# makezur/super_primitive

Hardware: AMD Instinct MI355X
Metric: GN iters/sec (640x480x64-seg frame pairs) (higher is better)
Workload: dtype f32; 1 GPU; Replica-shaped two-frame SfM, 640x480, 64 segments (grid, 4 px overlap), pyramid level 0 of a 3-level pyramid; BASELINE.json configs[1]; pairs_per_gpu=384, segment_pixels_per_pair=373056, optimiser=gn, tile_points=8192, span_points=4096, granule=64

## Files before the change

include/sp_hip.h:

```cpp
#ifndef SP_HIP_H
#define SP_HIP_H

#include <stdint.h>

#ifdef __cplusplus
extern "C" {
#endif

#define SP_ABI_VERSION 18

#define SP_EINVAL (-1)
#define SP_ELIMIT (-2)

#define SP_GRAD_PARTIAL_FLOATS 16
#define SP_GN_PARTIAL_FLOATS   32
#define SP_GNA_PARTIAL_FLOATS  48

int sp_abi_version(void);


int sp_mask_count(const uint8_t* masks, int N, int H, int W, int32_t* row_counts, int32_t* counts,
                  int32_t* seg_off, void* stream);

int sp_table_fill(const uint8_t* masks, const float* logdepth, const float* keypoints, int N, int H, int W,
                  const int32_t* seg_off, const int32_t* row_off, uint32_t* pix, float* baseL, float* kp_L,
                  void* stream);

int sp_table_sample_source(uint32_t* pix, const float* baseL, const int32_t* seg_off, const float* kp_L,
                           const float* kld, int N, int P, int H, int W, const float* img, int Hl, int Wl,
                           const float* K, float* src4, int set_validity, void* stream);

int sp_pack_rgb(const float* chw, int B, int H, int W, float* hwc3, void* stream);

int sp_blur_decimate(const float* in, int C, int H, int W, float* out, void* stream);

#define SP_PREP_MAX_STRIDES 4
#define SP_PREP_MAX_LEVELS 4
typedef struct SpPrepTable {
    const uint8_t* masks;
    const float* logdepth;
    const float* keypoints;
    float* kp_L;
    int32_t* row_counts[SP_PREP_MAX_STRIDES];
    int32_t* counts[SP_PREP_MAX_STRIDES];
    const int32_t* seg_off[SP_PREP_MAX_STRIDES];
    uint32_t* pix[SP_PREP_MAX_STRIDES];
    float* baseL[SP_PREP_MAX_STRIDES];
    int32_t stride[SP_PREP_MAX_STRIDES];
    int32_t N, H, W, n_strides;
    uint32_t* bits;
    const int32_t* boxes;
} SpPrepTable;
typedef struct SpPrepSample {
    uint32_t* pix;
    const float* baseL;
    const int32_t* seg_off;
    const int32_t* counts;
    const float* kp_L;
    const float* kld;
    const float* K;
    const float* image[SP_PREP_MAX_LEVELS];
    float* src4[SP_PREP_MAX_LEVELS];
    int32_t Hl[SP_PREP_MAX_LEVELS], Wl[SP_PREP_MAX_LEVELS];
    int32_t N, P, H, W, n_levels;
    int32_t granule;
} SpPrepSample;
#define SP_PREP_DEPTH_TABLE 0x10000
#define SP_PREP_DENSE_L 0x20000
typedef struct SpPrepImage {
    const float* in;
    float* out;
    int32_t H, W;
} SpPrepImage;
int sp_prepare_count(const SpPrepTable* tables, int n_tables, int max_rows, int max_N, void* stream);
int sp_prepare_count_boxed(const SpPrepTable* tables, int n_tables, int max_rows, int max_N, void* stream);
int sp_prepare_fill(const SpPrepTable* tables, int n_tables, int max_rows, int max_N, void* stream);
int sp_prepare_sample(const SpPrepSample* jobs, int n_jobs, int max_P, void* stream);
int sp_prepare_sample_pairs(const SpPrepSample* jobs_a, int max_P_a, const SpPrepSample* jobs_b, int max_P_b, int n_jobs, void* stream);
int sp_prepare_blur(const SpPrepImage* jobs, int n_jobs, int C, int max_out_pixels, void* stream);
int sp_prepare_pack(const SpPrepImage* jobs, int n_jobs, int max_pixels, void* stream);
typedef struct SpPrepImagePack {
    const float* in;
    float* out;
    float* packed_in;
    float* packed_out;
    int32_t H, W;
} SpPrepImagePack;
int sp_prepare_blur_pack(const SpPrepImagePack* jobs, int n_jobs, int max_out_pixels, void* stream);
int sp_prepare_gather(const float* const* src, const long long* off, int n, float* out, void* stream);

int sp_photo_cost_grad(const uint32_t* pix, const float* src4, const int32_t* seg_off, const float* kp_L,
                       const int32_t* tiles, const int32_t* seg_tile_off, int n_tiles, int N, int P, int H, int W,
                       const float* K_src, const float* kld, const float* trg3, int Hl, int Wl,
                       const float* K_trg, const float* pose, int B, const float* aff_src, const float* aff_trg,
                       float zmin, float* workspace, float* residual, float* g_kld, float* g_pose, float* g_aff,
                       void* stream);

int sp_points_workspace_floats(int n_points, int B);
int sp_points_cost_grad(const float* xyz, const float* rgb, int n_points, int P_total, int H, int W, const float* trg3,
                        int Hl, int Wl, const float* K_trg, const float* pose, int B, const float* aff_src,
                        const float* aff_trg, float zmin, float* workspace, float* residual, float* g_pose, float* g_aff,
                        void* stream);

int sp_photo_stats(const uint32_t* pix, const float* src4, const int32_t* seg_off, const float* kp_L, int N, int P,
                   int H, int W, const float* K_src, const float* kld, const float* trg3, int Hl, int Wl,
                   const float* K_trg, const float* pose, int B, const float* aff_src, const float* aff_trg,
                   float zmin, float* src_pts, float* trg_pts, float* src_rgb, float* trg_rgb, float* raw,
                   uint8_t* src_valid, uint8_t* trg_valid, int64_t* seg_ids, int stride, void* stream);

#define SP_GRAD_SEG_FLOATS 1
#define SP_GN_SEG_FLOATS 12
#define SP_GNA_SEG_FLOATS 12
typedef struct SpPair {
    const uint32_t* pix;
    const float*    src4;
    const float*    kp_L;
    const float*    trg3;
    float*          kld;
    float*          pose;
    float*          aff;
    const int32_t*  seg_tile_off;
    float K_src[4];
    float K_trg[4];
    int32_t N, P, H, W, Hl, Wl;
    int32_t tile0;
    int32_t n_tiles;
    float zmin;
    int32_t rec0;
} SpPair;

int sp_host_work_list_chunks(const long long* pc, int n_segs, int tile_points, int granule);
int sp_host_layout(const int32_t* counts, int n_lattices, int n_segs, const long long* n_off, int n_pairs, int granule,
                   long long* pc, long long* seg_pos, long long* p_off, int32_t* seg_off, long long* points);
int sp_host_work_list(const long long* pc, const long long* seg_pos, const long long* n_off, int n_pairs, int span_points,
                      int tile_points, int granule , int records_per_chunk ,
                      int32_t* chunks, int32_t* spans, int32_t* seg_tile_off, long long* sto_off, long long* c_off, long long* s_off);

#define SP_COST_WAVE_SPANS 0x100
#define SP_COST_DEPTH_TABLE 0x200

int sp_pairs_cost(const SpPair* pairs, const int32_t* chunks, const int32_t* spans, int n_spans, int mode, float irls_eps,
                  float* span_partials, float* seg_partials, void* stream);
struct SpRunDesc;
int sp_pairs_cost_opt(const SpPair* pairs, const int32_t* chunks, const int32_t* spans, int n_spans, int mode, float irls_eps,
                      float* span_partials, float* seg_partials, const int32_t* done, const uint32_t* pix_base,
                      const struct SpRunDesc* desc, void* stream);

int sp_pairs_adam_step(const SpPair* pairs, int n_pairs, int max_N, const float* span_partials, const float* seg_partials,
                       float lr_kld, float lr_pose, float lr_aff, float* state, float* losses, void* stream);

#define SP_LM_STATE_FLOATS 8
int sp_pairs_gn_step(const SpPair* pairs, int n_pairs, int max_N, const float* span_partials, const float* seg_partials,
                     float lm_up, float lm_down, float lm_min, float* lm_state, float* backup, float* costs, void* stream);

int sp_pairs_gn_step_conv(const SpPair* pairs, int n_pairs, int max_N, const float* span_partials, const float* seg_partials,
                          float lm_up, float lm_down, float lm_min, float* lm_state, float* backup, float* costs, float conv_tol,
                          int32_t* done, void* stream);

typedef struct SpRunDesc {
    uint32_t valid[2];
    float d[2];
    float base[2];
    float k;
    int32_t runs;
} SpRunDesc;

int sp_run_desc_build(const uint32_t* pix, int n_groups, SpRunDesc* desc, int32_t* n_general, void* stream);

#define SP_MAX_PHASES 12
#define SP_PHASE_POSE_ONLY 1
#define SP_PHASE_WAVE_SPANS 2
#define SP_PHASE_DEPTH_TABLE 4
#define SP_PHASE_DEPTH_DAMP_SHIFT 8
#define SP_PHASE_DEPTH_DAMP(k) (((k) & 0xff) << SP_PHASE_DEPTH_DAMP_SHIFT)
#define SP_PHASE_ADAM 8
#define SP_PHASE_PREDICTED_EXIT 16
typedef struct SpPhase {
    const SpPair* pairs;
    const int32_t* chunks;
    const int32_t* spans;
    float* span_partials;
    float* seg_partials;
    int32_t n_spans;
    int32_t max_iters;
    float irls_eps;
    float conv_tol;
    int32_t flags;
    int32_t next;
} SpPhase;
typedef struct SpSchedule {
    SpPhase phase[SP_MAX_PHASES];
    int32_t n_phases;
    int32_t entry;
    int32_t retry_entry;
    int32_t retry2_entry;
    float adam_lr_pose, adam_lr_kld;
    float* adam_state;
} SpSchedule;

#define SP_STATUS_NONFINITE   1
#define SP_STATUS_LAST_CAP    2
#define SP_STATUS_DEPTH_RANGE 4
#define SP_STATUS_COST        8
#define SP_STATUS_VALID       16
#define SP_STATUS_SEGMENTS    32
#define SP_STATUS_RETRIED     0x100
#define SP_STATUS_ADAM        0x400
#define SP_STATUS_UNFINISHED  0x200
#define SP_DIAG_FLOATS 8
typedef struct SpVerdict {
    int32_t* status;
    float* diag;
    int32_t* attempts;
    const float* pose0;
    const float* kld0;
    const float* pose_base;
    const float* kld_base;
    float kld_bound;
    float cost_bound;
    float cost_ratio;
    float valid_min;
    int32_t retry_mask;
    float lam0;
    float seg_max_ratio;
    float seg_mean_ratio;
    int32_t* evals;
    float seg_product;
    float pad_;
} SpVerdict;
#define SP_VERDICT_SEGMENTS 2048
#define SP_VERDICT_SEGMENT_POINTS 64
#define SP_VERDICT_MIN_SEGMENTS 8
int sp_pairs_schedule_cost(const SpSchedule* sched, const int32_t* phase, void* stream);
int sp_pairs_schedule_gn_step(const SpSchedule* sched, int n_pairs, int max_N, float lm_up, float lm_down, float lm_min,
                              float* lm_state, float* backup, float* costs, int32_t* phase, int32_t* iters, const SpVerdict* verdict ,
                              void* stream);

int sp_pairs_schedule_run(const SpSchedule* sched, int n_pairs, int max_N, float lm_up, float lm_down, float lm_min,
                          float* lm_state, float* backup, float* costs, int32_t* phase, int32_t* iters, int check_every,
                          int max_rounds, int32_t* flag_dev, int32_t* flag_host, const SpVerdict* verdict , void* stream);

typedef struct SpQueue {
    const SpPair* qpairs[SP_MAX_PHASES];
    SpPair* slot_pairs[SP_MAX_PHASES];
    int32_t max_spans[SP_MAX_PHASES];
    int32_t n_queue;
    int32_t pad_;
    int32_t* head;
    int32_t* slot_pair;
    float* q_costs;
    float* q_lm;
    float lam0;
    int32_t pad2_;
    int32_t* active;
} SpQueue;
int sp_pairs_schedule_run_queue(const SpSchedule* sched, const SpQueue* queue, int n_slots, int max_N, float lm_up, float lm_down,
                                float lm_min, float* lm_state, float* backup, float* costs, int32_t* phase, int32_t* iters,
                                int check_every, int max_rounds, int32_t* flag_dev, int32_t* flag_host, const SpVerdict* verdict ,
                                void* stream);

int sp_pairs_adam_iterate(const SpPair* pairs, const int32_t* chunks, const int32_t* spans, int n_spans, int n_pairs, int max_N,
                          float* span_partials, float* seg_partials, int32_t* arrivals, float lr_kld, float lr_pose, float lr_aff, float* state,
                          float* losses, void* stream);
int sp_pairs_gn_iterate(const SpPair* pairs, const int32_t* chunks, const int32_t* spans, int n_spans, int n_pairs, int max_N,
                        float irls_eps, float* span_partials, float* seg_partials, int32_t* arrivals, float lm_up, float lm_down,
                        float lm_min,
                        float* lm_state, float* backup, float* costs, void* stream);

typedef struct SpWindowNode {
    float T[16];
    float a[6];
    float m[6], v[6];
    float aff[2];
    float aff_m[2], aff_v[2];
    float lr_pose;
    float lr_aff;
    int32_t kind;
    int32_t flags;
} SpWindowNode;

typedef struct SpWindowEdge {
    int32_t src_node;
    int32_t trg_node;
    int32_t block;
    float weight;
} SpWindowEdge;

typedef struct SpWindowBlock {
    float* kld;
    float* m;
    float* v;
    int32_t N;
    float lr;
} SpWindowBlock;

int sp_window_scratch_doubles(int n_edges, int max_N);

int sp_window_compose(const SpPair* pairs, const SpWindowEdge* edges, int n_edges, SpWindowNode* nodes, int n_nodes, void* stream);

int sp_window_step(const SpPair* pairs, const SpWindowEdge* edges, int n_edges, SpWindowNode* nodes, int n_nodes,
                   const SpWindowBlock* blocks, int n_blocks, int max_N, const float* span_partials, const float* seg_partials,
                   double* scratch, int abs_loss, int skip_first, float rel_tol, float* state, float* losses, int max_losses,
                   void* stream);

int sp_window_gn_scratch_doubles(int n_edges, int n_blocks, int sum_N, int max_N, int n_unknowns);
int sp_window_gn_profile_offset(int n_edges, int n_blocks, int sum_N, int max_N, int n_unknowns);
int sp_window_gn_step(const SpPair* pairs, const SpWindowEdge* edges, int n_edges, SpWindowNode* nodes, int n_nodes,
                      const SpWindowBlock* blocks, int n_blocks, int sum_N, int max_N, int n_unknowns, const float* span_partials,
                      const float* seg_partials, double* scratch, SpWindowNode* nodes_backup, float* kld_backup, int flags,
                      float lm_up, float lm_down, float lm_min, float conv_tol, float* state, float* losses, int max_losses,
                      void* stream);

typedef struct SpWindowGn {
    const SpPair* pairs;
    const int32_t* chunks;
    const int32_t* spans;
    const SpWindowEdge* edges;
    SpWindowNode* nodes;
    const SpWindowBlock* blocks;
    float* span_partials;
    float* seg_partials;
    double* scratch;
    SpWindowNode* nodes_backup;
    float* kld_backup;
    float* state;
    float* losses;
    int32_t n_spans, n_edges, n_nodes, n_blocks, sum_N, max_N, n_unknowns, max_losses;
} SpWindowGn;
int sp_window_gn_multi_bytes(void);
int sp_window_gn_run_multi(const SpWindowGn* windows, int n_windows, float irls_eps, int flags, float lm_up, float lm_down, float lm_min,
                           float conv_tol, int max_iters, int check_every, void* args_dev, float* states_dev, float* states_host, void* stream);

int sp_window_gn_run(const SpPair* pairs, const int32_t* chunks, const int32_t* spans, int n_spans, float irls_eps,
                     const SpWindowEdge* edges, int n_edges, SpWindowNode* nodes, int n_nodes, const SpWindowBlock* blocks, int n_blocks,
                     int sum_N, int max_N, int n_unknowns, float* span_partials, float* seg_partials, double* scratch,
                     SpWindowNode* nodes_backup, float* kld_backup, int flags, float lm_up, float lm_down, float lm_min, float conv_tol,
                     float* state, float* losses, int max_losses, int max_iters, int check_every, float* state_host, void* stream);


int sp_depth_expand(const uint8_t* masks, const float* logdepth, const float* keypoints, const float* kld, int N,
                    int H, int W, int log_space, float* out, void* stream);

int sp_depth_splat(const uint32_t* pix, const float* baseL, const int32_t* seg_off, const float* kp_L,
                   const float* kld, int N, int P, int H, int W, const float* K, const float* pose,
                   unsigned long long* keys, float* out, void* stream);

int sp_depth_splat_mean(const uint32_t* pix, const float* baseL, const int32_t* seg_off, const float* kp_L, const float* kld, int N,
                        int P, int H, int W, const float* K, const float* pose, void* acc, float* out, void* stream);

int sp_segment_reinit(const uint32_t* pix, const float* baseL, const int32_t* seg_off, const float* kp_L, int N,
                      int P, int H, int W, const float* est_depth, int mode, float* scratch, float* out_kld,
                      uint8_t* out_visible, void* stream);

int sp_depth_average(const uint32_t* pix, const float* baseL, const int32_t* seg_off, const float* kp_L,
                     const float* kld, const uint8_t* visible, int N, int P, int H, int W, void* acc,
                     float* out_depth, uint8_t* out_invalid, void* stream);

int sp_depth_accumulate(const uint32_t* pix, const float* baseL, const int32_t* seg_off, const float* kp_L,
                        const float* kld, const uint8_t* visible, int N, int P, int H, int W, void* acc, void* stream);
int sp_depth_average_finish(const void* acc, int H, int W, float* out_depth, uint8_t* out_invalid, void* stream);

int sp_se3_retract(const float* a, const float* X, int n, float* T, const float* grad_T, float* grad_a, void* stream);

int sp_renormalise_se3(float* T, int n, void* stream);


int sp_depth_discontinuity(const float* logdepth, const uint8_t* valid, int N, int H, int W, int filter_size,
                           float threshold, float* scratch, uint8_t* split, uint8_t* disc, void* stream);

int sp_label_components(const uint8_t* fg, int N, int H, int W, int32_t* parent, int32_t* labels, int32_t* sizes,
                        void* stream);

int sp_collect_parts(const int32_t* labels, const int32_t* sizes, const uint8_t* masks, const uint8_t* split, int N, int H,
                     int W, int cap, int32_t* parts, int32_t* n_parts, int32_t* bg_sizes, void* stream);

int sp_build_part_masks(const uint8_t* masks, const uint8_t* split, const int32_t* labels, int H, int W,
                        const int32_t* parts, int K, uint8_t* out, void* stream);

int sp_kth_mask_pixel(const uint8_t* masks, const int32_t* row_off, int K, int H, int W, const int32_t* kth,
                      int32_t* out_rc, void* stream);

int sp_normal_integration_plan_words(int N);
int sp_normal_integration_segment_floats(int H, int W);
int sp_normal_integration_plan(const uint8_t* masks, const int32_t* boxes_or_null, int N, int H, int W, int32_t* plan, void* stream);
int sp_normal_integration(const float* normals, const float* K, const uint8_t* masks, const int32_t* boxes_or_null, int N, int H,
                          int W, int cg_max_iter, float cg_tol, int flags, float* scratch, long long scratch_floats, float* depth,
                          float* info, void* stream);

int sp_depth_fill_workspace_bytes(int B, int H, int W);
int sp_depth_fill_nearest(const float* depth, const uint8_t* invalid, int B, int H, int W, void* workspace, float* filled,
                          int32_t* index_or_null, int32_t* counts, void* stream);
int sp_depth_metrics_workspace_doubles(int B, int H, int W);
int sp_depth_metrics(const float* estimate, const float* target, const uint8_t* valid, int B, int H, int W, double* workspace,
                     double* out, void* stream);

int sp_kf_criterion(const float* depth, int n, float thresh, const float* pose_src, const float* pose_trg, float* out,
                    void* stream);
int sp_kf_criterion_ws_words(void);
int sp_kf_criterion_ws(const float* depth, int n, float thresh, const float* pose_src, const float* pose_trg, uint32_t* ws, float* out,
                       void* stream);

#define SP_CHAIN_LEVELS 4
#define SP_CHAIN_PHASES 6
#define SP_CHAIN_TRACK 1
#define SP_CHAIN_SUPP 2
#define SP_CHAIN_CRITERION 4
typedef struct SpChainPhase {
    int32_t level;
    int32_t max_iters;
    float irls_eps, conv_tol;
} SpChainPhase;
typedef struct SpChainWindow {
    SpWindowGn gn[SP_CHAIN_LEVELS];
    SpChainPhase phase[SP_CHAIN_PHASES];
    int32_t n_phases;
    int32_t check_every;
    int32_t flags;
    float lam0;
    float lm_up, lm_down, lm_min;
    int32_t check_first;
    float* state_host;
} SpChainWindow;
typedef struct SpChainTarget {
    float* packed[SP_CHAIN_LEVELS];
    const float* pose;
    const float* aff;
    int32_t node;
    int32_t pad_;
} SpChainTarget;
typedef struct SpChainStep {
    int32_t stages;
    int32_t H, W, n_levels;
    const float* image;
    float* level[SP_CHAIN_LEVELS];
    SpChainWindow track;
    SpChainTarget track_target;
    float* out_pose;
    float* out_aff;
    SpChainWindow supp;
    SpChainTarget supp_target[2];
    int32_t supp_images;
    int32_t kld_n;
    const float* kld_src;
    float* kld_dst;
    const uint32_t* pix; const float* baseL; const int32_t* seg_off; const float* kp_L; const float* kld;
    const float* K; const float* kf_pose;
    int32_t N, P;
    unsigned long long* keys; float* depth_out;
    float* rel_pose;
    float* crit;
    uint32_t* crit_ws;
    float* crit_host;
    float valid_thresh;
    int32_t track_iters, supp_iters;
    int32_t pad_;
} SpChainStep;

int sp_chain_multi_bytes(void);
int sp_chain_step_multi(SpChainStep* steps, int n_steps, void* args_dev, float* states_dev, float* states_host, void* stream);

#ifdef __cplusplus
}
#endif
#endif
```

super_primitive_amd/_lib.py:

```python
from __future__ import annotations

import ctypes
import os
from ctypes import c_float, c_int, c_void_p

_HERE = os.path.dirname(os.path.abspath(__file__))
LIB_PATH = os.environ.get("SP_HIP_LIB") or os.path.join(_HERE, "csrc", "libsp_hip.so")

P = c_void_p
I = c_int
F = c_float

SIGNATURES = {
    "sp_abi_version": [],
    "sp_mask_count": [P, I, I, I, P, P, P, P],
    "sp_table_fill": [P, P, P, I, I, I, P, P, P, P, P, P],
    "sp_table_sample_source": [P, P, P, P, P, I, I, I, I, P, I, I, P, P, I, P],
    "sp_pack_rgb": [P, I, I, I, P, P],
    "sp_blur_decimate": [P, I, I, I, P, P],
    "sp_photo_cost_grad": [P, P, P, P, P, P, I, I, I, I, I, P, P, P, I, I, P, P, I, P, P, F, P, P, P, P, P, P],
    "sp_points_workspace_floats": [I, I],
    "sp_points_cost_grad": [P, P, I, I, I, I, P, I, I, P, P, I, P, P, F, P, P, P, P, P],
    "sp_photo_stats": [P, P, P, P, I, I, I, I, P, P, P, I, I, P, P, I, P, P, F, P, P, P, P, P, P, P, P, I, P],
    "sp_pairs_cost": [P, P, P, I, I, F, P, P, P],
    "sp_pairs_adam_step": [P, I, I, P, P, F, F, F, P, P, P],
    "sp_pairs_gn_step": [P, I, I, P, P, F, F, F, P, P, P, P],
    "sp_pairs_cost_opt": [P, P, P, I, I, F, P, P, P, P, P, P],
    "sp_run_desc_build": [P, I, P, P, P],
    "sp_pairs_gn_step_conv": [P, I, I, P, P, F, F, F, P, P, P, F, P, P],
    "sp_prepare_count": [P, I, I, I, P],
    "sp_prepare_count_boxed": [P, I, I, I, P],
    "sp_prepare_fill": [P, I, I, I, P],
    "sp_prepare_sample": [P, I, I, P],
    "sp_prepare_sample_pairs": [P, I, P, I, I, P],
    "sp_prepare_blur": [P, I, I, I, P],
    "sp_prepare_pack": [P, I, I, P],
    "sp_prepare_blur_pack": [P, I, I, P],
    "sp_prepare_gather": [P, P, I, P, P],
    "sp_host_work_list_chunks": [P, I, I, I],
    "sp_host_layout": [P, I, I, P, I, I, P, P, P, P, P],
    "sp_host_work_list": [P, P, P, I, I, I, I, I, P, P, P, P, P, P],
    "sp_pairs_schedule_cost": [P, P, P],
    "sp_pairs_schedule_gn_step": [P, I, I, F, F, F, P, P, P, P, P, P, P],
    "sp_pairs_schedule_run": [P, I, I, F, F, F, P, P, P, P, P, I, I, P, P, P, P],
    "sp_pairs_schedule_run_queue": [P, P, I, I, F, F, F, P, P, P, P, P, I, I, P, P, P, P],
    "sp_pairs_adam_iterate": [P, P, P, I, I, I, P, P, P, F, F, F, P, P, P],
    "sp_pairs_gn_iterate": [P, P, P, I, I, I, F, P, P, P, F, F, F, P, P, P, P],
    "sp_window_scratch_doubles": [I, I],
    "sp_window_compose": [P, P, I, P, I, P],
    "sp_window_step": [P, P, I, P, I, P, I, I, P, P, P, I, I, F, P, P, I, P],
    "sp_window_gn_scratch_doubles": [I, I, I, I, I],
    "sp_window_gn_profile_offset": [I, I, I, I, I],
    "sp_window_gn_run": [P, P, P, I, F, P, I, P, I, P, I, I, I, I, P, P, P, P, P, I, F, F, F, F, P, P, I, I, I, P, P],
    "sp_window_gn_multi_bytes": [],
    "sp_window_gn_run_multi": [P, I, F, I, F, F, F, F, I, I, P, P, P, P],
    "sp_window_gn_step": [P, P, I, P, I, P, I, I, I, I, P, P, P, P, P, I, F, F, F, F, P, P, I, P],
    "sp_depth_expand": [P, P, P, P, I, I, I, I, P, P],
    "sp_depth_splat_mean": [P, P, P, P, P, I, I, I, I, P, P, P, P, P],
    "sp_depth_splat": [P, P, P, P, P, I, I, I, I, P, P, P, P, P],
    "sp_segment_reinit": [P, P, P, P, I, I, I, I, P, I, P, P, P, P],
    "sp_depth_average": [P, P, P, P, P, P, I, I, I, I, P, P, P, P],
    "sp_depth_accumulate": [P, P, P, P, P, P, I, I, I, I, P, P],
    "sp_depth_average_finish": [P, I, I, P, P, P],
    "sp_kf_criterion": [P, I, F, P, P, P, P],
    "sp_chain_multi_bytes": [],
    "sp_chain_step_multi": [P, I, P, P, P, P],
    "sp_kf_criterion_ws_words": [],
    "sp_kf_criterion_ws": [P, I, F, P, P, P, P, P],
    "sp_se3_retract": [P, P, I, P, P, P, P],
    "sp_renormalise_se3": [P, I, P],
    "sp_depth_discontinuity": [P, P, I, I, I, I, F, P, P, P, P],
    "sp_label_components": [P, I, I, I, P, P, P, P],
    "sp_collect_parts": [P, P, P, P, I, I, I, I, P, P, P, P],
    "sp_build_part_masks": [P, P, P, I, I, P, I, P, P],
    "sp_kth_mask_pixel": [P, P, I, I, I, P, P, P],
    "sp_normal_integration_plan_words": [I],
    "sp_normal_integration_segment_floats": [I, I],
    "sp_normal_integration_plan": [P, P, I, I, I, P, P],
    "sp_normal_integration": [P, P, P, P, I, I, I, I, F, I, P, ctypes.c_longlong, P, P, P],
    "sp_depth_fill_workspace_bytes": [I, I, I],
    "sp_depth_fill_nearest": [P, P, I, I, I, P, P, P, P, P],
    "sp_depth_metrics_workspace_doubles": [I, I, I],
    "sp_depth_metrics": [P, P, P, I, I, I, P, P, P],
}

SP_ABI_VERSION = 18
SP_GRAD_PARTIAL_FLOATS = 16
SP_GN_PARTIAL_FLOATS = 32
SP_GNA_PARTIAL_FLOATS = 48
SP_GNA_SEG_FLOATS = 12
SP_GRAD_SEG_FLOATS = 1
SP_GN_SEG_FLOATS = 12
SP_LM_STATE_FLOATS = 8


class SpPair(ctypes.Structure):
    _fields_ = [
        ("pix", c_void_p), ("src4", c_void_p), ("kp_L", c_void_p), ("trg3", c_void_p),
        ("kld", c_void_p), ("pose", c_void_p), ("aff", c_void_p), ("seg_tile_off", c_void_p),
        ("K_src", c_float * 4), ("K_trg", c_float * 4),
        ("N", c_int), ("P", c_int), ("H", c_int), ("W", c_int), ("Hl", c_int), ("Wl", c_int),
        ("tile0", c_int), ("n_tiles", c_int), ("zmin", c_float), ("rec0", c_int),
    ]


SP_MAX_PHASES = 12
SP_PHASE_POSE_ONLY = 1
SP_PHASE_WAVE_SPANS = 2
SP_COST_WAVE_SPANS = 0x100
SP_COST_DEPTH_TABLE = 0x200
SP_PHASE_DEPTH_TABLE = 4
SP_PHASE_ADAM = 8
SP_PHASE_PREDICTED_EXIT = 16
SP_PHASE_DEPTH_DAMP_SHIFT = 8
SP_PREP_DEPTH_TABLE = 0x10000
SP_PREP_DENSE_L = 0x20000


SP_PREP_MAX_STRIDES = 4
SP_PREP_MAX_LEVELS = 4


class SpPrepTable(ctypes.Structure):
    _fields_ = [("masks", c_void_p), ("logdepth", c_void_p), ("keypoints", c_void_p), ("kp_L", c_void_p),
                ("row_counts", c_void_p * SP_PREP_MAX_STRIDES), ("counts", c_void_p * SP_PREP_MAX_STRIDES),
                ("seg_off", c_void_p * SP_PREP_MAX_STRIDES), ("pix", c_void_p * SP_PREP_MAX_STRIDES),
                ("baseL", c_void_p * SP_PREP_MAX_STRIDES), ("stride", c_int * SP_PREP_MAX_STRIDES),
                ("N", c_int), ("H", c_int), ("W", c_int), ("n_strides", c_int), ("bits", c_void_p), ("boxes", c_void_p)]


class SpPrepSample(ctypes.Structure):
    _fields_ = [("pix", c_void_p), ("baseL", c_void_p), ("seg_off", c_void_p), ("counts", c_void_p), ("kp_L", c_void_p), ("kld", c_void_p),
                ("K", c_void_p), ("image", c_void_p * SP_PREP_MAX_LEVELS), ("src4", c_void_p * SP_PREP_MAX_LEVELS),
                ("Hl", c_int * SP_PREP_MAX_LEVELS), ("Wl", c_int * SP_PREP_MAX_LEVELS),
                ("N", c_int), ("P", c_int), ("H", c_int), ("W", c_int), ("n_levels", c_int), ("granule", c_int)]


class SpPrepImage(ctypes.Structure):
    _fields_ = [("inp", c_void_p), ("out", c_void_p), ("H", c_int), ("W", c_int)]


class SpPrepImagePack(ctypes.Structure):
    _fields_ = [("inp", c_void_p), ("out", c_void_p), ("packed_in", c_void_p), ("packed_out", c_void_p), ("H", c_int), ("W", c_int)]


class SpPhase(ctypes.Structure):
    _fields_ = [("pairs", c_void_p), ("chunks", c_void_p), ("spans", c_void_p), ("span_partials", c_void_p), ("seg_partials", c_void_p),
                ("n_spans", c_int), ("max_iters", c_int), ("irls_eps", c_float), ("conv_tol", c_float), ("flags", c_int), ("next", c_int)]


class SpSchedule(ctypes.Structure):
    _fields_ = [("phase", SpPhase * SP_MAX_PHASES), ("n_phases", c_int), ("entry", c_int), ("retry_entry", c_int), ("retry2_entry", c_int),
                ("adam_lr_pose", c_float), ("adam_lr_kld", c_float), ("adam_state", c_void_p)]


SP_STATUS_NONFINITE = 1
SP_STATUS_LAST_CAP = 2
SP_STATUS_DEPTH_RANGE = 4
SP_STATUS_COST = 8
SP_STATUS_VALID = 16
SP_STATUS_SEGMENTS = 32
SP_STATUS_RETRIED = 0x100
SP_STATUS_UNFINISHED = 0x200
SP_STATUS_ADAM = 0x400
SP_STATUS_FAILED = SP_STATUS_NONFINITE | SP_STATUS_LAST_CAP | SP_STATUS_DEPTH_RANGE | SP_STATUS_COST | SP_STATUS_VALID | SP_STATUS_SEGMENTS | SP_STATUS_UNFINISHED
SP_VERDICT_SEGMENTS = 2048
SP_VERDICT_SEGMENT_POINTS = 64
SP_VERDICT_MIN_SEGMENTS = 8
SP_DIAG_FLOATS = 8


class SpVerdict(ctypes.Structure):
    _fields_ = [("status", c_void_p), ("diag", c_void_p), ("attempts", c_void_p), ("pose0", c_void_p), ("kld0", c_void_p),
                ("pose_base", c_void_p), ("kld_base", c_void_p), ("kld_bound", c_float), ("cost_bound", c_float), ("cost_ratio", c_float),
                ("valid_min", c_float), ("retry_mask", c_int), ("lam0", c_float), ("seg_max_ratio", c_float), ("seg_mean_ratio", c_float), ("evals", c_void_p),
                ("seg_product", c_float), ("pad_", c_float)]


class SpQueue(ctypes.Structure):
    _fields_ = [("qpairs", c_void_p * SP_MAX_PHASES), ("slot_pairs", c_void_p * SP_MAX_PHASES), ("max_spans", c_int * SP_MAX_PHASES),
                ("n_queue", c_int), ("pad_", c_int),
                ("head", c_void_p), ("slot_pair", c_void_p), ("q_costs", c_void_p), ("q_lm", c_void_p), ("lam0", c_float), ("pad2_", c_int),
                ("active", c_void_p)]


class SpWindowGn(ctypes.Structure):
    _fields_ = [("pairs", c_void_p), ("chunks", c_void_p), ("spans", c_void_p), ("edges", c_void_p), ("nodes", c_void_p), ("blocks", c_void_p),
                ("span_partials", c_void_p), ("seg_partials", c_void_p), ("scratch", c_void_p), ("nodes_backup", c_void_p), ("kld_backup", c_void_p),
                ("state", c_void_p), ("losses", c_void_p), ("n_spans", c_int), ("n_edges", c_int), ("n_nodes", c_int), ("n_blocks", c_int),
                ("sum_N", c_int), ("max_N", c_int), ("n_unknowns", c_int), ("max_losses", c_int)]


SP_CHAIN_LEVELS, SP_CHAIN_PHASES = 4, 6
SP_CHAIN_TRACK, SP_CHAIN_SUPP, SP_CHAIN_CRITERION = 1, 2, 4


class SpChainPhase(ctypes.Structure):
    _fields_ = [("level", c_int), ("max_iters", c_int), ("irls_eps", c_float), ("conv_tol", c_float)]


class SpChainWindow(ctypes.Structure):
    _fields_ = [("gn", SpWindowGn * SP_CHAIN_LEVELS), ("phase", SpChainPhase * SP_CHAIN_PHASES), ("n_phases", c_int), ("check_every", c_int),
                ("flags", c_int), ("lam0", c_float), ("lm_up", c_float), ("lm_down", c_float), ("lm_min", c_float), ("check_first", c_int),
                ("state_host", c_void_p)]


class SpChainTarget(ctypes.Structure):
    _fields_ = [("packed", c_void_p * SP_CHAIN_LEVELS), ("pose", c_void_p), ("aff", c_void_p), ("node", c_int), ("pad_", c_int)]


class SpChainStep(ctypes.Structure):
    _fields_ = [("stages", c_int), ("H", c_int), ("W", c_int), ("n_levels", c_int), ("image", c_void_p), ("level", c_void_p * SP_CHAIN_LEVELS),
                ("track", SpChainWindow), ("track_target", SpChainTarget), ("out_pose", c_void_p), ("out_aff", c_void_p),
                ("supp", SpChainWindow), ("supp_target", SpChainTarget * 2), ("supp_images", c_int), ("kld_n", c_int), ("kld_src", c_void_p),
                ("kld_dst", c_void_p),
                ("pix", c_void_p), ("baseL", c_void_p), ("seg_off", c_void_p), ("kp_L", c_void_p), ("kld", c_void_p), ("K", c_void_p),
                ("kf_pose", c_void_p), ("N", c_int), ("P", c_int), ("keys", c_void_p), ("depth_out", c_void_p), ("rel_pose", c_void_p),
                ("crit", c_void_p), ("crit_ws", c_void_p), ("crit_host", c_void_p), ("valid_thresh", c_float), ("track_iters", c_int), ("supp_iters", c_int),
                ("pad_", c_int)]


class SpWindowNode(ctypes.Structure):
    _fields_ = [("T", c_float * 16), ("a", c_float * 6), ("m", c_float * 6), ("v", c_float * 6), ("aff", c_float * 2),
                ("aff_m", c_float * 2), ("aff_v", c_float * 2), ("lr_pose", c_float), ("lr_aff", c_float),
                ("kind", c_int), ("flags", c_int)]


class SpWindowEdge(ctypes.Structure):
    _fields_ = [("src_node", c_int), ("trg_node", c_int), ("block", c_int), ("weight", c_float)]


class SpWindowBlock(ctypes.Structure):
    _fields_ = [("kld", c_void_p), ("m", c_void_p), ("v", c_void_p), ("N", c_int), ("lr", c_float)]


_lib = None


def load():
    global _lib
    if _lib is not None:
        return _lib
    if not os.path.exists(LIB_PATH):
        raise RuntimeError(
            f"{LIB_PATH} not found: build it with `python -c 'import __graft_entry__ as g; g.build()'` "
            "(hipcc --offload-arch=gfx950).  There is no CPU / PyTorch fallback for the hot path.")
    try:
        import torch
    except Exception:
        pass
    lib = ctypes.CDLL(LIB_PATH)
    for name, args in SIGNATURES.items():
        fn = getattr(lib, name)
        fn.argtypes = args
        fn.restype = c_int
    if lib.sp_abi_version() != SP_ABI_VERSION:
        raise RuntimeError("libsp_hip.so ABI version mismatch; rebuild")
    _lib = lib
    return lib


def check(rc, what):
    if rc != 0:
        kind = {-1: "SP_EINVAL (bad argument)", -2: "SP_ELIMIT (size not supported)"}.get(rc, f"hipError_t {rc}")
        raise RuntimeError(f"{what} failed: {kind}")


def ptr(t):
    return None if t is None else ctypes.c_void_p(t.data_ptr())


_raw_stream = None


def stream_ptr():
    global _raw_stream
    if _raw_stream is None:
        import torch
        raw, cur = getattr(torch._C, "_cuda_getCurrentRawStream", None), getattr(torch._C, "_cuda_getDevice", None)
        if raw is not None and cur is not None:
            _raw_stream = lambda: raw(cur())
        else:
            _raw_stream = lambda: torch.cuda.current_stream().cuda_stream
    return ctypes.c_void_p(_raw_stream())


def require_device(*tensors):
    import torch
    dev = None
    for t in tensors:
        if t is None:
            continue
        if not t.is_cuda:
            raise RuntimeError("super_primitive_amd: the photometric hot path is HIP-only; got a CPU tensor. "
                               "Move the keyframe to a cuda device (no CPU fallback exists).")
        if dev is None:
            dev = t.device
        elif t.device != dev:
            raise RuntimeError(f"super_primitive_amd: operands on different devices ({dev} and {t.device})")
    if dev is not None and dev.index is not None and dev.index != torch.cuda.current_device():
        raise RuntimeError(f"super_primitive_amd: operands live on {dev} but the current device is "
                           f"cuda:{torch.cuda.current_device()}; wrap the call in `with torch.cuda.device({dev.index}):` "
                           "(one process per GPU is the supported layout)")
```

super_primitive_amd/csrc/sp_solve_device.h:

```cpp
#pragma once
#include "sp_device.h"

#define SP_LM_STRIDE SP_LM_STATE_FLOATS

template <int NV>
__device__ __forceinline__ void reduce_columns(const float* __restrict__ p, int n_tiles, double* out, double* scratch) {
    constexpr int G = SP_BLOCK / NV;
    const int g = threadIdx.x / NV, c = threadIdx.x - g * NV;
    if (g < G) {
        double s = 0.0;
        for (int t = g; t < n_tiles; t += 8 * G) {
            float v[8];
#pragma unroll
            for (int u = 0; u < 8; ++u) {
                const int tt = t + u * G;
                const float x = p[(size_t)min(tt, n_tiles - 1) * NV + c];
                v[u] = tt < n_tiles ? x : 0.f;
            }
#pragma unroll
            for (int u = 0; u < 8; ++u) s += (double)v[u];
        }
        scratch[g * NV + c] = s;
    }
    __syncthreads();
    if (threadIdx.x < NV) {
        double s = 0.0;
#pragma unroll
        for (int k = 0; k < G; ++k) s += scratch[k * NV + threadIdx.x];
        out[threadIdx.x] = s;
    }
    __syncthreads();
}

__device__ void se3_retract_left(const double xi[6], float* T16) {
    const double wx = xi[3], wy = xi[4], wz = xi[5];
    const double th2 = wx * wx + wy * wy + wz * wz;
    double A, B, C;
    if (th2 < 1e-12) {
        A = 1.0 - th2 / 6.0; B = 0.5 - th2 / 24.0; C = 1.0 / 6.0 - th2 / 120.0;
    } else if (th2 < 1e-4) {
        A = 1.0 - th2 / 6.0 * (1.0 - th2 / 20.0);
        B = 0.5 - th2 / 24.0 * (1.0 - th2 / 30.0);
        C = 1.0 / 6.0 - th2 / 120.0 * (1.0 - th2 / 42.0);
    } else {
        const double th = sqrt(th2);
        const double sn = sin(th), cs = cos(th);
        A = sn / th; B = (1.0 - cs) / th2; C = (th - sn) / (th2 * th);
    }
    const double W[9] = {0, -wz, wy, wz, 0, -wx, -wy, wx, 0};
    double W2[9];
    for (int i = 0; i < 3; ++i)
        for (int j = 0; j < 3; ++j) W2[3 * i + j] = W[3 * i] * W[j] + W[3 * i + 1] * W[3 + j] + W[3 * i + 2] * W[6 + j];
    double E[9], V[9];
    for (int i = 0; i < 9; ++i) {
        const double I = (i % 4 == 0) ? 1.0 : 0.0;
        E[i] = I + A * W[i] + B * W2[i];
        V[i] = I + B * W[i] + C * W2[i];
    }
    double dt[3];
    for (int i = 0; i < 3; ++i) dt[i] = V[3 * i] * xi[0] + V[3 * i + 1] * xi[1] + V[3 * i + 2] * xi[2];
    double R[9], t[3];
    for (int i = 0; i < 3; ++i) {
        for (int j = 0; j < 3; ++j) R[3 * i + j] = T16[4 * i + j];
        t[i] = T16[4 * i + 3];
    }
    for (int i = 0; i < 3; ++i) {
        for (int j = 0; j < 3; ++j)
            T16[4 * i + j] = (float)(E[3 * i] * R[j] + E[3 * i + 1] * R[3 + j] + E[3 * i + 2] * R[6 + j]);
        T16[4 * i + 3] = (float)(E[3 * i] * t[0] + E[3 * i + 1] * t[1] + E[3 * i + 2] * t[2] + dt[i]);
    }
    T16[12] = 0.f; T16[13] = 0.f; T16[14] = 0.f; T16[15] = 1.f;
}

__device__ __forceinline__ float adam_torch(float g, float& m, float& v, float neg_step, float bc2s) {
    m = m + 0.1f * (g - m);
    v = v * 0.999f;
    v = v + 0.001f * g * g;
    const float denom = sqrtf(v) / bc2s + 1e-8f;
    return neg_step * (m / denom);
}

struct AdamArgs {
    int max_N;
    float lr_kld, lr_pose, lr_aff;
    float* state;
    float* losses;
};

__device__ __forceinline__ void solve_adam(const SpPair* __restrict__ pairs, int pi, const float* __restrict__ partials,
                                           const float* __restrict__ seg_partials, const AdamArgs& h) {
    const int max_N = h.max_N;
    const float lr_kld = h.lr_kld, lr_pose = h.lr_pose, lr_aff = h.lr_aff;
    float* __restrict__ state = h.state;
    float* __restrict__ losses = h.losses;
    constexpr int NV = SP_GRAD_PARTIAL_FLOATS;
    __shared__ double sums[NV];
    __shared__ double scratch[(SP_BLOCK / NV) * NV];
    const SpPair& pr = pairs[pi];
    const float* p = partials + (size_t)pr.tile0 * NV;
    reduce_columns<NV>(p, pr.n_tiles, sums, scratch);
    const double scale = 1.0 / (3.0 * (double)pr.P);
    const float residual = (float)(sums[0] * scale);
    const double up = residual > 0.f ? scale : (residual < 0.f ? -scale : 0.0);
    float* st = state + (size_t)pi * (2 + 2 * (max_N + 8));
    float* m_kld = st + 2; float* v_kld = m_kld + max_N;
    float* m_xi = v_kld + max_N; float* v_xi = m_xi + 6;
    float* m_af = v_xi + 6; float* v_af = m_af + 2;
    const float step = st[0] + 1.f;
    const double bc1 = 1.0 - pow(0.9, (double)step);
    const float bc2s = (float)sqrt(1.0 - pow(0.999, (double)step));
    const float ns_kld = (float)(-(double)lr_kld / bc1), ns_pose = (float)(-(double)lr_pose / bc1), ns_aff = (float)(-(double)lr_aff / bc1);
    __syncthreads();
    for (int n = threadIdx.x; n < pr.N; n += SP_BLOCK) {
        double s = 0.0;
        const float* sp = seg_partials + (size_t)pr.rec0 * SP_GRAD_SEG_FLOATS;
        const int t0 = pr.seg_tile_off[n], t1 = pr.seg_tile_off[n + 1];
        for (int t = t0; t < t1; t += 8) {
            float v[8];
#pragma unroll
            for (int u = 0; u < 8; ++u) v[u] = sp[(size_t)min(t + u, t1 - 1) * SP_GRAD_SEG_FLOATS];
#pragma unroll
            for (int u = 0; u < 8; ++u) s += (t + u < t1) ? (double)v[u] : 0.0;
        }
        const float g = (float)(s * up);
        pr.kld[n] += adam_torch(g, m_kld[n], v_kld[n], ns_kld, bc2s);
    }
    if (threadIdx.x == 0) {
        double gR[9], gt[3], R[9], t[3];
        for (int i = 0; i < 3; ++i) {
            gt[i] = sums[1 + i] * up;
            for (int j = 0; j < 3; ++j) { gR[3 * i + j] = sums[4 + 3 * i + j] * up; R[3 * i + j] = pr.pose[4 * i + j]; }
            t[i] = pr.pose[4 * i + 3];
        }
        double A[9];
        for (int i = 0; i < 3; ++i)
            for (int j = 0; j < 3; ++j)
                A[3 * i + j] = R[3 * i] * gR[3 * j] + R[3 * i + 1] * gR[3 * j + 1] + R[3 * i + 2] * gR[3 * j + 2] + t[i] * gt[j];
        const float g6[6] = {(float)gt[0], (float)gt[1], (float)gt[2],
                             (float)(A[5] - A[7]), (float)(A[6] - A[2]), (float)(A[1] - A[3])};
        double xi[6];
        for (int i = 0; i < 6; ++i) xi[i] = adam_torch(g6[i], m_xi[i], v_xi[i], ns_pose, bc2s);
        se3_retract_left(xi, pr.pose);
        if (pr.aff) {
            const float ga = (float)(sums[14] * up), gb = (float)(sums[15] * up);
            pr.aff[2] += adam_torch(ga, m_af[0], v_af[0], ns_aff, bc2s);
            pr.aff[3] += adam_torch(gb, m_af[1], v_af[1], ns_aff, bc2s);
        }
        st[0] = step;
        losses[pi] = fabsf(residual);
    }
}


__device__ bool ldlt6_solve(double S[36], double rhs[6]) {
    double dinv[6];
    for (int j = 0; j < 6; ++j) {
        double d = S[7 * j];
        for (int k = 0; k < j; ++k) d -= S[6 * j + k] * S[6 * j + k] * S[7 * k];
        if (!(d > 0.0)) return false;
        S[7 * j] = d;
        dinv[j] = 1.0 / d;
        for (int i = j + 1; i < 6; ++i) {
            double v = S[6 * i + j];
            for (int k = 0; k < j; ++k) v -= S[6 * i + k] * S[6 * j + k] * S[7 * k];
            S[6 * i + j] = v * dinv[j];
        }
    }
    for (int i = 0; i < 6; ++i) {
        double v = rhs[i];
        for (int k = 0; k < i; ++k) v -= S[6 * i + k] * rhs[k];
        rhs[i] = v;
    }
    for (int i = 0; i < 6; ++i) rhs[i] *= dinv[i];
    for (int i = 5; i >= 0; --i) {
        double v = rhs[i];
        for (int k = i + 1; k < 6; ++k) v -= S[6 * k + i] * rhs[k];
        rhs[i] = v;
    }
    return true;
}

#define SP_SEG_CACHE 256

__device__ __forceinline__ void segment_system(const float* __restrict__ p, const int32_t* __restrict__ seg_tile_off, int n,
                                               double lam, double (&o)[8], bool pose_only = false) {
    constexpr int NV = SP_GN_SEG_FLOATS;
    if (pose_only) {
#pragma unroll
        for (int i = 0; i < 8; ++i) o[i] = 0.0;
        return;
    }
    double h[6] = {0, 0, 0, 0, 0, 0}, D = 0.0, bd = 0.0;
    const int t0 = seg_tile_off[n], t1 = seg_tile_off[n + 1];
    for (int t = t0; t < t1; t += 8) {
        float v[8][8];
#pragma unroll
        for (int u = 0; u < 8; ++u) {
            const float4* q = reinterpret_cast<const float4*>(p + (size_t)min(t + u, t1 - 1) * NV);
            const float4 a = q[0], b = q[1];
            v[u][0] = a.x; v[u][1] = a.y; v[u][2] = a.z; v[u][3] = a.w;
            v[u][4] = b.x; v[u][5] = b.y; v[u][6] = b.z; v[u][7] = b.w;
        }
#pragma unroll
        for (int u = 0; u < 8; ++u) {
            if (t + u < t1) {
#pragma unroll
                for (int i = 0; i < 6; ++i) h[i] += (double)v[u][i];
                D += (double)v[u][6];
                bd += (double)v[u][7];
            }
        }
    }
    const double Dd = D * (1.0 + lam);
#pragma unroll
    for (int i = 0; i < 6; ++i) o[i] = h[i];
    o[6] = Dd > 1e-12 ? 1.0 / Dd : 0.0;
    o[7] = bd;
}

struct GnArgs {
    int max_N;
    float lm_up, lm_down, lm_min;
    float* lm_state;
    float* backup;
    float* costs;
    float conv_tol;
    int32_t* done;
    int32_t* phase;
    int32_t* iters;
    int max_iters;
    int pose_only;
    int next_phase;
    float depth_damp;
    float adam_lr_pose, adam_lr_kld;
    float* adam_state;
    int predicted_exit;
    uint32_t idle_mask;
};

__device__ __forceinline__ void leave_phase(const GnArgs& h, int pi, float* __restrict__ ls, int spent, bool on_cap) {
    h.phase[pi] = h.next_phase;
    h.iters[pi] = 0;
    ls[1] = -1.f;
    ls[7] = on_cap ? (float)spent : -(float)spent;
}

__device__ __forceinline__ void solve_gn(const SpPair* __restrict__ pairs, int pi, const float* __restrict__ partials,
                                         const float* __restrict__ seg_partials, const GnArgs& h) {
    const int max_N = h.max_N;
    const float lm_up = h.lm_up, lm_down = h.lm_down, lm_min = h.lm_min;
    float* __restrict__ lm_state = h.lm_state;
    float* __restrict__ backup = h.backup;
    float* __restrict__ costs = h.costs;
    constexpr int NV = SP_GN_PARTIAL_FLOATS;
    __shared__ double sums[NV];
    __shared__ double scratch[(SP_BLOCK / NV) * NV];
    __shared__ double seg[SP_SEG_CACHE][8];
    __shared__ double schur_part[8][27];
    __shared__ double schur[27];
    __shared__ double dxi[6];
    __shared__ double gain_part[SP_WAVES];
    __shared__ int decision;
    const SpPair& pr = pairs[pi];
    if (h.done && h.done[pi]) return;
    const float* p = partials + (size_t)pr.tile0 * NV;
    const float* sp = seg_partials + (size_t)pr.rec0 * SP_GN_SEG_FLOATS;
    float* ls = lm_state + (size_t)pi * SP_LM_STRIDE;
    float* bk = backup + (size_t)pi * (16 + max_N);
    reduce_columns<NV>(p, pr.n_tiles, sums, scratch);
    const double cost = sums[0] / (3.0 * (double)pr.P);
    if (threadIdx.x == 0) {
        const float last = ls[1];
        int rej = 0;
        if (last >= 0.f && (float)cost > last * (1.f + 1e-6f) && ls[4] == 0.f) rej = 1;
        if (!rej && (h.done || h.phase) && h.conv_tol > 0.f && last >= 0.f && ls[4] == 0.f && (last - (float)cost) <= h.conv_tol * last) {
            rej = 2;
            if (h.done) h.done[pi] = 1;
            if (h.phase) { leave_phase(h, pi, ls, h.iters[pi], false); ls[4] = 0.f; }
        }
        decision = rej;
        ls[5] = (float)cost;
        ls[6] = (float)(sums[28] / (double)pr.P);
        costs[pi] = (float)cost;
    }
    __syncthreads();
    if (decision == 2) return;
    if (decision == 1) {
        for (int i = threadIdx.x; i < 16; i += SP_BLOCK) pr.pose[i] = bk[i];
        for (int n = threadIdx.x; n < pr.N; n += SP_BLOCK) pr.kld[n] = bk[16 + n];
        if (threadIdx.x == 0) {
            ls[0] *= lm_up; ls[3] += 1.f; ls[4] = 1.f;
            if (h.phase) {
                const int n = h.iters[pi] + 1;
                if (n >= h.max_iters) { leave_phase(h, pi, ls, n, true); ls[4] = 0.f; }
                else h.iters[pi] = n;
            }
        }
        return;
    }
    float lambda = ls[0];
    if (ls[4] == 0.f) lambda = fmaxf(lambda * lm_down, lm_min);
    const double lam = (double)lambda;
    for (int i = threadIdx.x; i < 16; i += SP_BLOCK) bk[i] = pr.pose[i];
    for (int n = threadIdx.x; n < pr.N; n += SP_BLOCK) bk[16 + n] = pr.kld[n];
    const int n_cached = min(pr.N, SP_SEG_CACHE);
    for (int n = threadIdx.x; n < n_cached; n += SP_BLOCK) {
        double o[8];
        segment_system(sp, pr.seg_tile_off, n, lam + (double)h.depth_damp, o, h.pose_only != 0);
#pragma unroll
        for (int i = 0; i < 8; ++i) seg[n][i] = o[i];
    }
    __syncthreads();
    {
        const int k = threadIdx.x >> 3, j = threadIdx.x & 7;
        if (k < 27) {
            int a = 0, b = 0;
            if (k < 21) { int rem = k, row = 0; while (rem >= 6 - row) { rem -= 6 - row; ++row; } a = row; b = row + rem; }
            else a = k - 21;
            double acc = 0.0;
            for (int n = j; n < pr.N; n += 8) {
                double o[8];
                if (n < SP_SEG_CACHE) {
#pragma unroll
                    for (int i = 0; i < 8; ++i) o[i] = seg[n][i];
                } else segment_system(sp, pr.seg_tile_off, n, lam + (double)h.depth_damp, o, h.pose_only != 0);
                acc += o[a] * (k < 21 ? o[b] : o[7]) * o[6];
            }
            schur_part[j][k] = acc;
        }
    }
    __syncthreads();
    if (threadIdx.x < 27) {
        double v = 0.0;
#pragma unroll
        for (int j = 0; j < 8; ++j) v += schur_part[j][threadIdx.x];
        schur[threadIdx.x] = v;
    }
    __syncthreads();
    if (threadIdx.x == 0) {
        double S[36], rhs[6];
        int k = 0;
        for (int i = 0; i < 6; ++i)
            for (int j = i; j < 6; ++j) {
                double v = sums[1 + k] - schur[k];
                if (i == j) v += lam * sums[1 + k] + 1e-12;
                S[6 * i + j] = v; S[6 * j + i] = v;
                ++k;
            }
        for (int i = 0; i < 6; ++i) rhs[i] = -(sums[22 + i] - schur[21 + i]);
        const bool ok = ldlt6_solve(S, rhs);
        for (int i = 0; i < 6; ++i) dxi[i] = ok ? rhs[i] : 0.0;
        ls[0] = lambda; ls[1] = (float)cost; ls[2] += 1.f; ls[4] = 0.f;
    }
    __syncthreads();
    double gain = 0.0;
    for (int n = threadIdx.x; n < pr.N; n += SP_BLOCK) {
        double o[8];
        if (n < SP_SEG_CACHE) {
#pragma unroll
            for (int i = 0; i < 8; ++i) o[i] = seg[n][i];
        } else segment_system(sp, pr.seg_tile_off, n, lam + (double)h.depth_damp, o, h.pose_only != 0);
        if (o[6] > 0.0) {
            double r = -o[7];
#pragma unroll
            for (int i = 0; i < 6; ++i) r -= o[i] * dxi[i];
            double dd = r * o[6];
            dd = fmin(fmax(dd, -0.5), 0.5);
            pr.kld[n] += (float)dd;
            gain -= o[7] * dd;
        }
    }
    if (threadIdx.x == 64) {
        double xi[6];
        for (int i = 0; i < 6; ++i) xi[i] = dxi[i];
        se3_retract_left(xi, pr.pose);
    }
    if (h.phase) {
#pragma unroll
        for (int o = 32; o > 0; o >>= 1) gain += __shfl_xor(gain, o, 64);
        if ((threadIdx.x & 63) == 0) gain_part[threadIdx.x >> 6] = gain;
        __syncthreads();
        if (threadIdx.x == 0) {
            const int n = h.iters[pi] + 1;
            bool done = false;
            if (h.predicted_exit && h.conv_tol > 0.f && h.depth_damp == 0.f && lambda <= 1e-2f) {
                double g = gain_part[0] + gain_part[1] + gain_part[2] + gain_part[3];
                for (int i = 0; i < 6; ++i) g -= sums[22 + i] * dxi[i];
                done = g / (3.0 * (double)pr.P) <= (double)h.conv_tol * cost;
            }
            if (done) leave_phase(h, pi, ls, n, false);
            else if (n >= h.max_iters) leave_phase(h, pi, ls, n, true);
            else h.iters[pi] = n;
        }
    }
}

__device__ __forceinline__ void solve_adam_sched(const SpPair* __restrict__ pairs, int pi, const float* __restrict__ partials,
                                                 const float* __restrict__ seg_partials, const GnArgs& h) {
    constexpr int NV = SP_GN_PARTIAL_FLOATS;
    __shared__ double sums[NV];
    __shared__ double scratch[(SP_BLOCK / NV) * NV];
    const SpPair& pr = pairs[pi];
    const int max_N = h.max_N;
    const float* p = partials + (size_t)pr.tile0 * NV;
    const float* sp = seg_partials + (size_t)pr.rec0 * SP_GN_SEG_FLOATS;
    float* ls = h.lm_state + (size_t)pi * SP_LM_STRIDE;
    reduce_columns<NV>(p, pr.n_tiles, sums, scratch);
    const double scale = 1.0 / (3.0 * (double)pr.P);
    float* st = h.adam_state + (size_t)pi * (2 + 2 * (max_N + 8));
    float* m_kld = st + 2; float* v_kld = m_kld + max_N;
    float* m_xi = v_kld + max_N; float* v_xi = m_xi + 6;
    const float step = st[0] + 1.f;
    const double bc1 = 1.0 - pow(0.9, (double)step);
    const float bc2s = (float)sqrt(1.0 - pow(0.999, (double)step));
    const float ns_kld = (float)(-(double)h.adam_lr_kld / bc1), ns_pose = (float)(-(double)h.adam_lr_pose / bc1);
    __syncthreads();
    for (int n = threadIdx.x; n < pr.N; n += SP_BLOCK) {
        double o[8];
        segment_system(sp, pr.seg_tile_off, n, 0.0, o);
        const float g = (float)(o[7] * scale);
        pr.kld[n] += adam_torch(g, m_kld[n], v_kld[n], ns_kld, bc2s);
    }
    if (threadIdx.x == 0) {
        double xi[6];
        for (int i = 0; i < 6; ++i) xi[i] = adam_torch((float)(sums[22 + i] * scale), m_xi[i], v_xi[i], ns_pose, bc2s);
        se3_retract_left(xi, pr.pose);
        st[0] = step;
        const float cost = (float)(sums[0] * scale);
        ls[1] = cost; ls[2] += 1.f; ls[4] = 0.f; ls[5] = cost;
        ls[6] = (float)(sums[28] / (double)pr.P);
        h.costs[pi] = cost;
        const int n = h.iters[pi] + 1;
        if (n >= h.max_iters) leave_phase(h, pi, ls, n, true);
        else h.iters[pi] = n;
    }
}

__device__ __forceinline__ void renormalise_rotation(float* __restrict__ M) {
    const float m00 = M[0], m01 = M[1], m02 = M[2], m10 = M[4], m11 = M[5], m12 = M[6], m20 = M[8], m21 = M[9], m22 = M[10];
    float q0 = 1.f + m00 + m11 + m22, q1 = 1.f + m00 - m11 - m22, q2 = 1.f - m00 + m11 - m22, q3 = 1.f - m00 - m11 + m22;
    q0 = q0 > 0.f ? sqrtf(q0) : 0.f; q1 = q1 > 0.f ? sqrtf(q1) : 0.f;
    q2 = q2 > 0.f ? sqrtf(q2) : 0.f; q3 = q3 > 0.f ? sqrtf(q3) : 0.f;
    int best = 0; float qb = q0;
    if (q1 > qb) { best = 1; qb = q1; }
    if (q2 > qb) { best = 2; qb = q2; }
    if (q3 > qb) { best = 3; qb = q3; }
    const float a = m21 - m12, b = m02 - m20, c = m10 - m01, d = m10 + m01, e = m02 + m20, f = m12 + m21;
    const float c0 = best == 0 ? q0 * q0 : (best == 1 ? a : (best == 2 ? b : c));
    const float c1 = best == 0 ? a : (best == 1 ? q1 * q1 : (best == 2 ? d : e));
    const float c2 = best == 0 ? b : (best == 1 ? d : (best == 2 ? q2 * q2 : f));
    const float c3 = best == 0 ? c : (best == 1 ? e : (best == 2 ? f : q3 * q3));
    const float den = 2.f * fmaxf(qb, 0.1f);
    const float r = c0 / den, x = c1 / den, y = c2 / den, z = c3 / den;
    const float s = 2.f / (r * r + x * x + y * y + z * z);
    M[0] = 1.f - s * (y * y + z * z); M[1] = s * (x * y - z * r);       M[2] = s * (x * z + y * r);
    M[4] = s * (x * y + z * r);       M[5] = 1.f - s * (x * x + z * z); M[6] = s * (y * z - x * r);
    M[8] = s * (x * z - y * r);       M[9] = s * (y * z + x * r);       M[10] = 1.f - s * (x * x + y * y);
}

template <int ND>
struct Dual {
    float v;
    float d[ND];
};
template <int ND> __device__ __forceinline__ Dual<ND> dconst(float c) { Dual<ND> r; r.v = c; for (int i = 0; i < ND; ++i) r.d[i] = 0.f; return r; }
template <int ND> __device__ __forceinline__ Dual<ND> operator+(const Dual<ND>& a, const Dual<ND>& b) { Dual<ND> r; r.v = a.v + b.v; for (int i = 0; i < ND; ++i) r.d[i] = a.d[i] + b.d[i]; return r; }
template <int ND> __device__ __forceinline__ Dual<ND> operator-(const Dual<ND>& a, const Dual<ND>& b) { Dual<ND> r; r.v = a.v - b.v; for (int i = 0; i < ND; ++i) r.d[i] = a.d[i] - b.d[i]; return r; }
template <int ND> __device__ __forceinline__ Dual<ND> operator-(const Dual<ND>& a) { Dual<ND> r; r.v = -a.v; for (int i = 0; i < ND; ++i) r.d[i] = -a.d[i]; return r; }
template <int ND> __device__ __forceinline__ Dual<ND> operator*(const Dual<ND>& a, const Dual<ND>& b) { Dual<ND> r; r.v = a.v * b.v; for (int i = 0; i < ND; ++i) r.d[i] = a.d[i] * b.v + a.v * b.d[i]; return r; }
template <int ND> __device__ __forceinline__ Dual<ND> operator*(float a, const Dual<ND>& b) { Dual<ND> r; r.v = a * b.v; for (int i = 0; i < ND; ++i) r.d[i] = a * b.d[i]; return r; }
template <int ND> __device__ __forceinline__ Dual<ND> chain(const Dual<ND>& a, float f, float df) { Dual<ND> r; r.v = f; for (int i = 0; i < ND; ++i) r.d[i] = df * a.d[i]; return r; }

template <int ND>
__device__ void se3_exp_times(const Dual<ND> (&a)[6], const float* __restrict__ X16, Dual<ND> (&T)[12]) {
    const Dual<ND> th2 = a[3] * a[3] + a[4] * a[4] + a[5] * a[5];
    const float t2 = th2.v;
    float A, B, C, dA, dB, dC;
    {
        const double t = (double)t2;
        double a_, b_, c_, da_, db_, dc_;
        if (t < 0.5) {
            double ia[10], ib[10], ic[10];
            {
                double f = 1.0;
                for (int k = 0; k < 10; ++k) {
                    const double n1 = 2.0 * k + 1.0;
                    if (k > 0) f *= (2.0 * k) * n1;
                    ia[k] = 1.0 / f; ib[k] = ia[k] / (n1 + 1.0); ic[k] = ib[k] / (n1 + 2.0);
                }
            }
            double va = 0.0, vb = 0.0, vc = 0.0, wa = 0.0, wb = 0.0, wc = 0.0;
            for (int k = 9; k >= 0; --k) {
                const double sg = (k & 1) ? -1.0 : 1.0;
                wa = wa * t + va; va = va * t + sg * ia[k];
                wb = wb * t + vb; vb = vb * t + sg * ib[k];
                wc = wc * t + vc; vc = vc * t + sg * ic[k];
            }
            a_ = va; b_ = vb; c_ = vc; da_ = wa; db_ = wb; dc_ = wc;
        } else {
            const double th = sqrt(t), sn = sin(th), cs = cos(th);
            a_ = sn / th; b_ = (1.0 - cs) / t; c_ = (th - sn) / (t * th);
            da_ = (cs * th - sn) / (2.0 * t * th);
            db_ = (sn * th - 2.0 * (1.0 - cs)) / (2.0 * t * t);
            dc_ = ((1.0 - cs) * th - 3.0 * (th - sn)) / (2.0 * t * t * th);
        }
        A = (float)a_; B = (float)b_; C = (float)c_; dA = (float)da_; dB = (float)db_; dC = (float)dc_;
    }
    const Dual<ND> dA_ = chain(th2, A, dA), dB_ = chain(th2, B, dB), dC_ = chain(th2, C, dC);
    const Dual<ND> z = dconst<ND>(0.f), one = dconst<ND>(1.f);
    const Dual<ND> W[9] = {z, -a[5], a[4], a[5], z, -a[3], -a[4], a[3], z};
    Dual<ND> W2[9];
    for (int i = 0; i < 3; ++i)
        for (int j = 0; j < 3; ++j) W2[3 * i + j] = W[3 * i] * W[j] + W[3 * i + 1] * W[3 + j] + W[3 * i + 2] * W[6 + j];
    Dual<ND> E[9], V[9];
    for (int i = 0; i < 9; ++i) {
        const Dual<ND> I = (i % 4 == 0) ? one : z;
        E[i] = I + dA_ * W[i] + dB_ * W2[i];
        V[i] = I + dB_ * W[i] + dC_ * W2[i];
    }
    for (int i = 0; i < 3; ++i) {
        const Dual<ND> dt = V[3 * i] * a[0] + V[3 * i + 1] * a[1] + V[3 * i + 2] * a[2];
        for (int j = 0; j < 3; ++j)
            T[4 * i + j] = X16[j] * E[3 * i] + X16[4 + j] * E[3 * i + 1] + X16[8 + j] * E[3 * i + 2];
        T[4 * i + 3] = X16[3] * E[3 * i] + X16[7] * E[3 * i + 1] + X16[11] * E[3 * i + 2] + dt;
    }
}
```

super_primitive_amd/csrc/sp_solver.hip:

```cpp
#include "sp_solve_device.h"

namespace {

__global__ __launch_bounds__(SP_BLOCK) void k_pairs_adam(const SpPair* __restrict__ pairs, const float* __restrict__ partials,
                                                         const float* __restrict__ seg_partials, AdamArgs h) {
    solve_adam(pairs, blockIdx.x, partials, seg_partials, h);
}

__global__ __launch_bounds__(SP_BLOCK) void k_pairs_gn(const SpPair* __restrict__ pairs, const float* __restrict__ partials,
                                                       const float* __restrict__ seg_partials, GnArgs h) {
    solve_gn(pairs, blockIdx.x, partials, seg_partials, h);
}

static_assert(sizeof(SpPhase) == 64 && sizeof(SpSchedule) == 800 && sizeof(SpVerdict) == 104 && sizeof(SpQueue) == 296 && sizeof(SpPair) == 136,
              "SpSchedule / SpVerdict / SpQueue / SpPair are part of the ABI");

__global__ __launch_bounds__(SP_BLOCK) void k_pairs_gn_sched(SpSchedule sched, GnArgs h, SpQueue q, SpVerdict v, const int32_t* __restrict__ active) {
    const int slot = active ? active[blockIdx.x] : blockIdx.x;
    const int ph = h.phase[slot];
    if (ph >= sched.n_phases || ph < 0) return;
    if ((h.idle_mask >> ph) & 1u) return;
    if (v.evals && threadIdx.x == 0) v.evals[(size_t)(q.n_queue > 0 ? q.slot_pair[slot] : slot) * SP_MAX_PHASES + ph] += 1;
    {
        const SpPhase& s = sched.phase[ph];
        h.conv_tol = s.conv_tol;
        h.max_iters = s.max_iters;
        h.pose_only = s.flags & SP_PHASE_POSE_ONLY;
        h.next_phase = s.next > 0 ? s.next : ph + 1;
        h.depth_damp = 0.125f * (float)((s.flags >> SP_PHASE_DEPTH_DAMP_SHIFT) & 0xff);
        h.adam_lr_pose = sched.adam_lr_pose; h.adam_lr_kld = sched.adam_lr_kld; h.adam_state = sched.adam_state;
        h.predicted_exit = s.flags & SP_PHASE_PREDICTED_EXIT;
        if ((s.flags & SP_PHASE_ADAM) && sched.adam_state) solve_adam_sched(s.pairs, slot, s.span_partials, s.seg_partials, h);
        else solve_gn(s.pairs, slot, s.span_partials, s.seg_partials, h);
    }
    if (q.n_queue <= 0 && !v.status) return;
    __shared__ int next_s, retry_s;
    __shared__ float dmax_s[SP_WAVES];
    __shared__ int bad_s[SP_WAVES];
    __shared__ float segc_s[SP_VERDICT_SEGMENTS];
    __shared__ float seg_med_s, seg_max_s[SP_WAVES];
    __shared__ int seg_n_s[SP_WAVES];
    __syncthreads();
    const int pid = q.n_queue > 0 ? q.slot_pair[slot] : slot;
    float* ls = h.lm_state + (size_t)slot * SP_LM_STRIDE;
    if (v.diag && threadIdx.x == 0) {
        float* first = v.diag + (size_t)pid * SP_DIAG_FLOATS + 5;
        if (*first == 0.f) *first = h.costs[slot];
    }
    if (h.phase[slot] < sched.n_phases) return;
    if (v.status) {
        const SpPair& pr = sched.phase[ph].pairs[slot];
        const float* kld0 = v.kld0 + (pr.kld - v.kld_base);
        const float* pose0 = v.pose0 + (pr.pose - v.pose_base);
        float dmax = 0.f;
        int bad = 0;
        for (int n = threadIdx.x; n < pr.N; n += SP_BLOCK) {
            const float d = fabsf(pr.kld[n] - kld0[n]);
            if (!(d <= 3.0e38f)) bad = 1;
            else dmax = fmaxf(dmax, d);
        }
        if (threadIdx.x < 12 && !(fabsf(pr.pose[threadIdx.x]) <= 3.0e38f)) bad = 1;
        const int n_seg = min(pr.N, SP_VERDICT_SEGMENTS);
        float smax = 0.f;
        int sn = 0;
        {
            const float* sp = sched.phase[ph].seg_partials + (size_t)pr.rec0 * SP_GN_SEG_FLOATS;
            for (int n = threadIdx.x; n < n_seg; n += SP_BLOCK) {
                double a = 0.0, c = 0.0;
                for (int t = pr.seg_tile_off[n]; t < pr.seg_tile_off[n + 1]; ++t) {
                    a += (double)sp[(size_t)t * SP_GN_SEG_FLOATS + 8];
                    c += (double)sp[(size_t)t * SP_GN_SEG_FLOATS + 9];
                }
                const float sc = c >= (double)SP_VERDICT_SEGMENT_POINTS ? (float)(a / (3.0 * c)) : -1.f;
                segc_s[n] = sc;
                if (sc >= 0.f) { smax = fmaxf(smax, sc); ++sn; }
            }
        }
#pragma unroll
        for (int o = 32; o > 0; o >>= 1) {
            dmax = fmaxf(dmax, __shfl_xor(dmax, o, 64)); bad |= __shfl_xor(bad, o, 64);
            smax = fmaxf(smax, __shfl_xor(smax, o, 64)); sn += __shfl_xor(sn, o, 64);
        }
        if ((threadIdx.x & 63) == 0) { dmax_s[threadIdx.x >> 6] = dmax; bad_s[threadIdx.x >> 6] = bad; seg_max_s[threadIdx.x >> 6] = smax; seg_n_s[threadIdx.x >> 6] = sn; }
        if (threadIdx.x == 0) seg_med_s = 0.f;
        __syncthreads();
        {
            const int n_judged = seg_n_s[0] + seg_n_s[1] + seg_n_s[2] + seg_n_s[3];
            const int want = (n_judged - 1) >> 1;
            for (int n = threadIdx.x; n < n_seg && n_judged >= SP_VERDICT_MIN_SEGMENTS; n += SP_BLOCK) {
                const float x = segc_s[n];
                if (x < 0.f) continue;
                int rank = 0;
                for (int j = 0; j < n_seg; ++j) {
                    const float y = segc_s[j];
                    rank += (y >= 0.f && (y < x || (y == x && j < n))) ? 1 : 0;
                }
                if (rank == want) seg_med_s = x;
            }
        }
        __syncthreads();
        if (threadIdx.x == 0) {
            dmax = fmaxf(fmaxf(dmax_s[0], dmax_s[1]), fmaxf(dmax_s[2], dmax_s[3]));
            bad = bad_s[0] | bad_s[1] | bad_s[2] | bad_s[3];
            const float cost = ls[5], first = v.diag ? v.diag[(size_t)pid * SP_DIAG_FLOATS + 5] : 0.f;
            int st = 0;
            if (bad || !(fabsf(cost) <= 3.0e38f)) st |= SP_STATUS_NONFINITE;
            if (ls[7] > 0.f) st |= SP_STATUS_LAST_CAP;
            if (v.kld_bound > 0.f && dmax > v.kld_bound) st |= SP_STATUS_DEPTH_RANGE;
            if ((v.cost_bound > 0.f && cost > v.cost_bound) || (v.cost_ratio > 0.f && first > 0.f && cost > v.cost_ratio * first)) st |= SP_STATUS_COST;
            if (v.valid_min > 0.f && ls[6] < v.valid_min) st |= SP_STATUS_VALID;
            const float seg_med = seg_med_s, seg_max = fmaxf(fmaxf(seg_max_s[0], seg_max_s[1]), fmaxf(seg_max_s[2], seg_max_s[3]));
            if (seg_med > 0.f && ((v.seg_max_ratio > 0.f && seg_max > v.seg_max_ratio * seg_med) || (v.seg_mean_ratio > 0.f && cost > v.seg_mean_ratio * seg_med) ||
                                  (v.seg_product > 0.f && (cost / seg_med - 1.f) * (seg_max / seg_med) > v.seg_product)))
                st |= SP_STATUS_SEGMENTS;
            const int attempt = v.attempts ? v.attempts[pid] : 2;
            const bool failed = (st & v.retry_mask) != 0;
            const bool has1 = sched.retry_entry >= 0 && sched.retry_entry < sched.n_phases, has2 = sched.retry2_entry >= 0 && sched.retry2_entry < sched.n_phases;
            int again = 0;
            if (failed && attempt == 0 && has1) again = 1;
            else if (failed && attempt <= 1 && has2) again = 2;
            retry_s = again;
            if (again) {
                v.attempts[pid] = again;
                h.phase[slot] = again == 1 ? sched.retry_entry : sched.retry2_entry; h.iters[slot] = 0;
                ls[0] = v.lam0; ls[1] = -1.f; ls[4] = 0.f; ls[7] = 0.f;
                if (v.diag) v.diag[(size_t)pid * SP_DIAG_FLOATS + 5] = 0.f;
            } else {
                v.status[pid] = st | (attempt > 0 && v.attempts ? SP_STATUS_RETRIED : 0) | (attempt > 1 && v.attempts ? SP_STATUS_ADAM : 0);
                if (v.diag) {
                    float* d = v.diag + (size_t)pid * SP_DIAG_FLOATS;
                    d[0] = cost; d[1] = dmax; d[2] = ls[6]; d[3] = fabsf(ls[7]); d[4] = (float)(v.attempts ? attempt + 1 : 1); d[6] = seg_med; d[7] = seg_max;
                }
            }
        }
        __syncthreads();
        if (retry_s) {
            for (int n = threadIdx.x; n < pr.N; n += SP_BLOCK) pr.kld[n] = kld0[n];
            if (threadIdx.x < 16) pr.pose[threadIdx.x] = pose0[threadIdx.x];
            if (sched.adam_state) {
                float* st = sched.adam_state + (size_t)slot * (2 + 2 * (h.max_N + 8));
                for (int i = threadIdx.x; i < 2 + 2 * (h.max_N + 8); i += SP_BLOCK) st[i] = 0.f;
            }
            return;
        }
    }
    if (q.n_queue <= 0) return;
    if (threadIdx.x < SP_LM_STRIDE) q.q_lm[(size_t)pid * SP_LM_STRIDE + threadIdx.x] = ls[threadIdx.x];
    if (threadIdx.x == 0) {
        q.q_costs[pid] = h.costs[slot];
        next_s = atomicAdd(q.head, 1);
    }
    __syncthreads();
    const int next = next_s;
    if (next >= q.n_queue) return;
    {
        constexpr int WORDS = (int)(sizeof(SpPair) / sizeof(uint32_t));
        for (int i = threadIdx.x; i < sched.n_phases * WORDS; i += SP_BLOCK) {
            const int p = i / WORDS, k = i - p * WORDS;
            reinterpret_cast<uint32_t*>(q.slot_pairs[p] + slot)[k] = reinterpret_cast<const uint32_t*>(q.qpairs[p] + next)[k];
        }
    }
    if (sched.adam_state) {
        float* st = sched.adam_state + (size_t)slot * (2 + 2 * (h.max_N + 8));
        for (int i = threadIdx.x; i < 2 + 2 * (h.max_N + 8); i += SP_BLOCK) st[i] = 0.f;
    }
    if (threadIdx.x == 0) {
        h.phase[slot] = sched.entry; h.iters[slot] = 0;
        ls[0] = q.lam0; ls[1] = -1.f; ls[2] = 0.f; ls[3] = 0.f; ls[4] = 0.f; ls[5] = 0.f; ls[6] = 0.f; ls[7] = 0.f;
        q.slot_pair[slot] = next;
    }
}

__global__ void k_mark_unfinished(const int32_t* __restrict__ phase, const int32_t* __restrict__ slot_pair, int n_slots, int n_phases,
                                  int32_t* __restrict__ status) {
    const int i = blockIdx.x * blockDim.x + threadIdx.x;
    if (i < n_slots && phase[i] < n_phases) status[slot_pair ? slot_pair[i] : i] = SP_STATUS_UNFINISHED;
}

__global__ __launch_bounds__(SP_BLOCK) void k_phase_min(const int32_t* __restrict__ phase, int n, int32_t* __restrict__ out,
                                                        const int32_t* __restrict__ head, const int32_t* __restrict__ attempts,
                                                        const int32_t* __restrict__ slot_pair, int n_phases, int last_attempt,
                                                        int32_t* __restrict__ active_out) {
    __shared__ int part[SP_WAVES], first[SP_WAVES];
    __shared__ int n_active_s;
    __shared__ unsigned occ_s;
    if (threadIdx.x == 0) { n_active_s = 0; occ_s = 0u; }
    __syncthreads();
    int m = 0x7fffffff, f = 0;
    unsigned occ = 0u;
    for (int i = threadIdx.x; i < n; i += SP_BLOCK) {
        const int ph = phase[i];
        m = min(m, ph);
        if (ph >= 0 && ph < n_phases) { const int at = atomicAdd(&n_active_s, 1); if (active_out) active_out[at] = i; occ |= 1u << ph; }
        if (attempts && ph < n_phases && attempts[slot_pair ? slot_pair[i] : i] < last_attempt) f = 1;
    }
#pragma unroll
    for (int o = 32; o > 0; o >>= 1) { m = min(m, __shfl_xor(m, o, 64)); f |= __shfl_xor(f, o, 64); }
    if (occ) atomicOr(&occ_s, occ);
    if ((threadIdx.x & 63) == 0) { part[threadIdx.x >> 6] = m; first[threadIdx.x >> 6] = f; }
    __syncthreads();
    if (threadIdx.x == 0) {
        out[4] = (int32_t)occ_s;
        out[0] = min(min(part[0], part[1]), min(part[2], part[3]));
        out[1] = head ? *head : 0;
        out[2] = first[0] | first[1] | first[2] | first[3];
        out[3] = n_active_s;
    }
}

__global__ void k_renormalise(float* __restrict__ T, int n) {
    const int i = blockIdx.x * blockDim.x + threadIdx.x;
    if (i >= n) return;
    renormalise_rotation(T + 16 * (size_t)i);
}

__global__ void k_se3_retract(const float* __restrict__ a6, const float* __restrict__ X, int n, float* __restrict__ T,
                              const float* __restrict__ G, float* __restrict__ ga) {
    const int b = blockIdx.x * blockDim.x + threadIdx.x;
    if (b >= n) return;
    const float* a = a6 + 6 * (size_t)b;
    const float* Xb = X + 16 * (size_t)b;
    if (!G) {
        Dual<1> ad[6], out[12];
        for (int i = 0; i < 6; ++i) { ad[i].v = a[i]; ad[i].d[0] = 0.f; }
        se3_exp_times<1>(ad, Xb, out);
        float* Tb = T + 16 * (size_t)b;
        for (int i = 0; i < 12; ++i) Tb[i] = out[i].v;
        Tb[12] = 0.f; Tb[13] = 0.f; Tb[14] = 0.f; Tb[15] = 1.f;
    } else {
        Dual<6> ad[6], out[12];
        for (int i = 0; i < 6; ++i) { ad[i].v = a[i]; for (int k = 0; k < 6; ++k) ad[i].d[k] = (i == k) ? 1.f : 0.f; }
        se3_exp_times<6>(ad, Xb, out);
        const float* Gb = G + 16 * (size_t)b;
        for (int k = 0; k < 6; ++k) {
            float s = 0.f;
            for (int i = 0; i < 12; ++i) s = fmaf(out[i].d[k], Gb[i], s);
            ga[6 * (size_t)b + k] = s;
        }
    }
}

}

extern "C" {

int sp_pairs_adam_step(const SpPair* pairs, int n_pairs, int max_N, const float* partials, const float* seg_partials,
                       float lr_kld, float lr_pose, float lr_aff, float* state, float* losses, void* stream) {
    if (!pairs || !partials || !seg_partials || !state || !losses || n_pairs <= 0 || max_N <= 0) return SP_EINVAL;
    hipLaunchKernelGGL(k_pairs_adam, dim3(n_pairs), dim3(SP_BLOCK), 0, static_cast<hipStream_t>(stream), pairs, partials,
                       seg_partials, AdamArgs{max_N, lr_kld, lr_pose, lr_aff, state, losses});
    SP_CHECK_LAUNCH();
    return 0;
}

int sp_pairs_gn_step_conv(const SpPair* pairs, int n_pairs, int max_N, const float* partials, const float* seg_partials,
                          float lm_up, float lm_down, float lm_min, float* lm_state, float* backup, float* costs, float conv_tol,
                          int32_t* done, void* stream) {
    if (!pairs || !partials || !seg_partials || !lm_state || !backup || !costs || n_pairs <= 0 || max_N <= 0) return SP_EINVAL;
    if (conv_tol > 0.f && !done) return SP_EINVAL;
    hipLaunchKernelGGL(k_pairs_gn, dim3(n_pairs), dim3(SP_BLOCK), 0, static_cast<hipStream_t>(stream), pairs, partials,
                       seg_partials, GnArgs{max_N, lm_up, lm_down, lm_min, lm_state, backup, costs, conv_tol, done, nullptr, nullptr, 0, 0});
    SP_CHECK_LAUNCH();
    return 0;
}

static uint32_t adam_phases(const SpSchedule* sched) {
    uint32_t m = 0;
    for (int p = 0; p < sched->n_phases; ++p) if (sched->phase[p].flags & SP_PHASE_ADAM) m |= 1u << p;
    return m;
}

static int check_schedule(const SpSchedule* sched, const SpVerdict* v) {
    if (!sched || sched->n_phases <= 0 || sched->n_phases > SP_MAX_PHASES) return SP_EINVAL;
    if (sched->entry < 0 || sched->entry >= sched->n_phases || sched->retry_entry < -1 || sched->retry_entry >= sched->n_phases) return SP_EINVAL;
    if (sched->retry2_entry < -1 || sched->retry2_entry >= sched->n_phases) return SP_EINVAL;
    for (int p = 0; p < sched->n_phases; ++p) {
        const SpPhase& ph = sched->phase[p];
        if (!ph.pairs || !ph.span_partials || !ph.seg_partials || ph.max_iters <= 0) return SP_EINVAL;
        if ((ph.flags & SP_PHASE_ADAM) && (!sched->adam_state || !(sched->adam_lr_pose > 0.f) || !(sched->adam_lr_kld > 0.f))) return SP_EINVAL;
        if (ph.next != 0 && (ph.next <= p || ph.next > sched->n_phases)) return SP_EINVAL;
    }
    if (v && v->status) {
        if (!v->pose0 || !v->kld0 || !v->pose_base || !v->kld_base) return SP_EINVAL;
        if ((sched->retry_entry >= 0 || sched->retry2_entry >= 0) && v->retry_mask != 0 && !v->attempts) return SP_EINVAL;
    }
    return 0;
}

int sp_pairs_schedule_gn_step(const SpSchedule* sched, int n_pairs, int max_N, float lm_up, float lm_down, float lm_min,
                              float* lm_state, float* backup, float* costs, int32_t* phase, int32_t* iters, const SpVerdict* verdict,
                              void* stream) {
    if (!sched || !lm_state || !backup || !costs || !phase || !iters || n_pairs <= 0 || max_N <= 0) return SP_EINVAL;
    if (int rc = check_schedule(sched, verdict)) return rc;
    hipLaunchKernelGGL(k_pairs_gn_sched, dim3(n_pairs), dim3(SP_BLOCK), 0, static_cast<hipStream_t>(stream), *sched,
                       GnArgs{max_N, lm_up, lm_down, lm_min, lm_state, backup, costs, 0.f, nullptr, phase, iters, 0, 0, 0}, SpQueue{},
                       verdict ? *verdict : SpVerdict{}, (const int32_t*)nullptr);
    SP_CHECK_LAUNCH();
    return 0;
}

int sp_pairs_schedule_run_queue(const SpSchedule* sched, const SpQueue* queue, int n_slots, int max_N, float lm_up, float lm_down,
                                float lm_min, float* lm_state, float* backup, float* costs, int32_t* phase, int32_t* iters,
                                int check_every, int max_rounds, int32_t* flag_dev, int32_t* flag_host, const SpVerdict* verdict, void* stream) {
    if (!sched || !queue || !phase || !iters || !flag_dev || !flag_host || !lm_state || !backup || !costs) return SP_EINVAL;
    if (check_every <= 0 || max_rounds < 0 || n_slots <= 0 || max_N <= 0 || queue->n_queue < n_slots) return SP_EINVAL;
    if (int rc = check_schedule(sched, verdict)) return rc;
    if (!queue->head || !queue->slot_pair || !queue->q_costs || !queue->q_lm) return SP_EINVAL;
    for (int p = 0; p < sched->n_phases; ++p) {
        const SpPhase& ph = sched->phase[p];
        if (!queue->qpairs[p] || queue->slot_pairs[p] != ph.pairs || queue->max_spans[p] < 0) return SP_EINVAL;
        if ((ph.flags & SP_PHASE_WAVE_SPANS) && (queue->max_spans[p] & 3)) return SP_EINVAL;
        if ((long long)queue->max_spans[p] * n_slots > 0x7fffffffLL) return SP_ELIMIT;
    }
    hipStream_t s = static_cast<hipStream_t>(stream);
    const SpVerdict vd = verdict ? *verdict : SpVerdict{};
    const bool may_retry = vd.status && vd.attempts && vd.retry_mask != 0 && (sched->retry_entry >= 0 || sched->retry2_entry >= 0);
    const int last_attempt = sched->retry2_entry >= 0 ? 2 : 1;
    int it = 0;
    int reached = 0;
    int min_phase = 0;
    int n_active = 0;
    const uint32_t adam_mask = adam_phases(sched);
    uint32_t occupied = 1u << sched->entry;
    uint32_t seen = 0;
    while (it < max_rounds) {
        const bool tail = queue->active && n_active > 0 && 8 * n_active <= n_slots;
        const int every = (tail && seen != 0 && (seen & ~adam_mask) == 0) ? 4 * check_every : check_every;
        const int n = (max_rounds - it) < every ? (max_rounds - it) : every;
        const uint32_t idle = adam_mask & ~occupied;
        GnArgs ga{max_N, lm_up, lm_down, lm_min, lm_state, backup, costs, 0.f, nullptr, phase, iters, 0, 0, 0};
        ga.idle_mask = idle;
        for (int k = 0; k < n; ++k, ++it) {
            int rc = schedule_cost_from(sched, phase, stream, reached, queue, n_slots, tail ? queue->active : nullptr, tail ? n_active : 0, idle);
            if (rc != 0) return rc < 0 ? rc : -(1000 + rc);
            hipLaunchKernelGGL(k_pairs_gn_sched, dim3(tail ? n_active : n_slots), dim3(SP_BLOCK), 0, s, *sched, ga, *queue, vd,
                               tail ? (const int32_t*)queue->active : (const int32_t*)nullptr);
            hipError_t e = hipGetLastError();
            if (e != hipSuccess) return -(1000 + (int)e);
        }
        hipLaunchKernelGGL(k_phase_min, dim3(1), dim3(SP_BLOCK), 0, s, phase, n_slots, flag_dev, queue->head, may_retry ? vd.attempts : nullptr,
                           queue->slot_pair, sched->n_phases, last_attempt, queue->active);
        hipError_t e = hipGetLastError();
        if (e == hipSuccess) e = hipMemcpyAsync(flag_host, flag_dev, 5 * sizeof(int32_t), hipMemcpyDeviceToHost, s);
        if (e == hipSuccess) e = hipStreamSynchronize(s);
        if (e != hipSuccess) return -(1000 + (int)e);
        min_phase = static_cast<volatile int32_t*>(flag_host)[0];
        seen = (uint32_t)static_cast<volatile int32_t*>(flag_host)[4];
        occupied = seen | (1u << sched->entry);
        const int head = static_cast<volatile int32_t*>(flag_host)[1];
        n_active = head >= queue->n_queue ? static_cast<volatile int32_t*>(flag_host)[3] : 0;
        const bool first_attempts_left = static_cast<volatile int32_t*>(flag_host)[2] != 0;
        if (min_phase >= sched->n_phases) break;
        reached = (head >= queue->n_queue && !(may_retry && first_attempts_left)) ? (min_phase < 0 ? 0 : min_phase) : 0;
    }
    if (min_phase < sched->n_phases && vd.status) {
        hipLaunchKernelGGL(k_mark_unfinished, dim3((n_slots + 255) / 256), dim3(256), 0, s, phase, queue->slot_pair, n_slots, sched->n_phases, vd.status);
        hipError_t e = hipGetLastError();
        if (e != hipSuccess) return -(1000 + (int)e);
    }
    return it;
}

int sp_pairs_schedule_run(const SpSchedule* sched, int n_pairs, int max_N, float lm_up, float lm_down, float lm_min,
                          float* lm_state, float* backup, float* costs, int32_t* phase, int32_t* iters, int check_every,
                          int max_rounds, int32_t* flag_dev, int32_t* flag_host, const SpVerdict* verdict, void* stream) {
    if (!sched || !phase || !iters || !flag_dev || !flag_host || check_every <= 0 || max_rounds < 0) return SP_EINVAL;
    if (!lm_state || !backup || !costs || n_pairs <= 0 || max_N <= 0) return SP_EINVAL;
    if (int rc = check_schedule(sched, verdict)) return rc;
    hipStream_t s = static_cast<hipStream_t>(stream);
    const bool may_retry = verdict && verdict->status && verdict->attempts && verdict->retry_mask != 0 && (sched->retry_entry >= 0 || sched->retry2_entry >= 0);
    const int last_attempt = sched->retry2_entry >= 0 ? 2 : 1;
    int it = 0;
    int reached = 0;
    int min_phase = 0;
    const uint32_t adam_mask = adam_phases(sched);
    uint32_t occupied = 0xffffffffu;
    while (it < max_rounds) {
        const int n = (max_rounds - it) < check_every ? (max_rounds - it) : check_every;
        const uint32_t idle = adam_mask & ~occupied;
        for (int k = 0; k < n; ++k, ++it) {
            int rc = schedule_cost_from(sched, phase, stream, reached, nullptr, 0, nullptr, 0, idle);
            if (rc == 0) rc = check_schedule(sched, verdict);
            if (rc != 0) return rc < 0 ? rc : -(1000 + rc);
            GnArgs ga{max_N, lm_up, lm_down, lm_min, lm_state, backup, costs, 0.f, nullptr, phase, iters, 0, 0, 0};
            ga.idle_mask = idle;
            hipLaunchKernelGGL(k_pairs_gn_sched, dim3(n_pairs), dim3(SP_BLOCK), 0, s, *sched, ga, SpQueue{}, verdict ? *verdict : SpVerdict{}, (const int32_t*)nullptr);
            hipError_t el = hipGetLastError();
            if (el != hipSuccess) return -(1000 + (int)el);
        }
        hipLaunchKernelGGL(k_phase_min, dim3(1), dim3(SP_BLOCK), 0, s, phase, n_pairs, flag_dev, (const int32_t*)nullptr,
                           may_retry ? (const int32_t*)verdict->attempts : (const int32_t*)nullptr, (const int32_t*)nullptr, sched->n_phases, last_attempt,
                           (int32_t*)nullptr);
        hipError_t e = hipGetLastError();
        if (e == hipSuccess) e = hipMemcpyAsync(flag_host, flag_dev, 5 * sizeof(int32_t), hipMemcpyDeviceToHost, s);
        if (e == hipSuccess) e = hipStreamSynchronize(s);
        if (e != hipSuccess) return -(1000 + (int)e);
        reached = min_phase = static_cast<volatile int32_t*>(flag_host)[0];
        occupied = (uint32_t)static_cast<volatile int32_t*>(flag_host)[4];
        if (reached >= sched->n_phases) break;
        if (reached < 0 || (may_retry && static_cast<volatile int32_t*>(flag_host)[2] != 0)) reached = 0;
    }
    if (verdict && verdict->status && min_phase < sched->n_phases) {
        hipLaunchKernelGGL(k_mark_unfinished, dim3((n_pairs + 255) / 256), dim3(256), 0, s, phase, (const int32_t*)nullptr, n_pairs, sched->n_phases, verdict->status);
        hipError_t e = hipGetLastError();
        if (e != hipSuccess) return -(1000 + (int)e);
    }
    return it;
}

int sp_pairs_gn_step(const SpPair* pairs, int n_pairs, int max_N, const float* partials, const float* seg_partials,
                     float lm_up, float lm_down, float lm_min, float* lm_state, float* backup, float* costs, void* stream) {
    return sp_pairs_gn_step_conv(pairs, n_pairs, max_N, partials, seg_partials, lm_up, lm_down, lm_min, lm_state, backup, costs, 0.f,
                                 nullptr, stream);
}

int sp_renormalise_se3(float* T, int n, void* stream) {
    if (!T || n <= 0) return SP_EINVAL;
    hipLaunchKernelGGL(k_renormalise, dim3((n + 63) / 64), dim3(64), 0, static_cast<hipStream_t>(stream), T, n);
    SP_CHECK_LAUNCH();
    return 0;
}

int sp_se3_retract(const float* a, const float* X, int n, float* T, const float* grad_T, float* grad_a, void* stream) {
    if (!a || !X || n <= 0) return SP_EINVAL;
    if (grad_T ? !grad_a : !T) return SP_EINVAL;
    hipLaunchKernelGGL(k_se3_retract, dim3((n + 63) / 64), dim3(64), 0, static_cast<hipStream_t>(stream), a, X, n, T, grad_T,
                       grad_a);
    SP_CHECK_LAUNCH();
    return 0;
}

}
```

super_primitive_amd/optim/pair_batch.py:

```python
from __future__ import annotations

import ctypes

import numpy as np
import torch

from .. import _lib
from ..image import gaussian_pyramid
from . import batch_prepare

_SP_PAIR_DTYPE = np.dtype(_lib.SpPair)

DEFAULT_BATCH_TILE_POINTS = 8192
DEFAULT_SPAN_POINTS = 16384
MIN_SPANS = 2304
GRANULE = 256

FRAME_PAIR_POINT_STRIDE = (2, 2, 4)
FRAME_PAIR_SCHEDULE = dict(max_iters_per_level=25, conv_tol=2e-3, polish_max=15, polish_eps=1e-5, polish_tol=1e-4, check_every=3, predicted_exit=True)
FIXED_FRAME_PAIR_SCHEDULE = dict(iters_per_level=15, polish_iters=10, polish_eps=1e-5)
REFERENCE_START_LEVELS = (0, 3)
REFERENCE_START_POINT_STRIDE = (2, 2, 4)
REFERENCE_START_RETRY = (dict(level=2, stride=4, max_iters=30, irls_eps=1e-3, conv_tol=2e-3, pose_only=True),)
REFERENCE_START_ADAM = (dict(level=2, stride=4, max_iters=500, irls_eps=1e-5, conv_tol=0.0, adam=True),
                        dict(level=1, stride=2, max_iters=500, irls_eps=1e-5, conv_tol=0.0, adam=True),
                        dict(level=0, stride=2, max_iters=500, irls_eps=1e-5, conv_tol=0.0, adam=True))
ADAM_LR_POSE, ADAM_LR_KLD = 1e-2, 1e-3
REFERENCE_START_SCHEDULE = dict(FRAME_PAIR_SCHEDULE, pose_first_iters=15, pose_first_eps=1e-2, coarse_damped="auto", retry_phases=REFERENCE_START_RETRY,
                                retry2_phases=REFERENCE_START_ADAM)
COST_OUTLIER_MIN_PAIRS = 8
VERDICT_DEFAULTS = dict(kld_bound=2.0, cost_bound=0.0, cost_ratio=0.0, valid_min=0.5, cost_outlier=4.0, seg_max_ratio=8.0, seg_mean_ratio=1.3, seg_product=0.9,
                        retry_on=_lib.SP_STATUS_NONFINITE | _lib.SP_STATUS_LAST_CAP | _lib.SP_STATUS_DEPTH_RANGE | _lib.SP_STATUS_VALID | _lib.SP_STATUS_COST
                        | _lib.SP_STATUS_SEGMENTS)


def _level_images(img, max_level):
    out, cur = [img], img[None]
    for _ in range(max_level):
        cur = gaussian_pyramid.blur_decimate(cur)
        out.append(cur[0])
    return out


def pad_layout(counts, device):
    counts = np.asarray(counts, dtype=np.int64)
    pc = (counts + GRANULE - 1) // GRANULE * GRANULE
    pseg_off = np.concatenate(([0], np.cumsum(pc)))
    seg_off = np.concatenate(([0], np.cumsum(counts)))
    dst = torch.from_numpy(np.repeat(pseg_off[:-1] - seg_off[:-1], counts) + np.arange(int(counts.sum()))).to(device)
    return dict(pc=pc, pseg_off=pseg_off, Ppad=int(pseg_off[-1]), dst=dst)


def pad_points(x, pd):
    out = torch.zeros((pd['Ppad'],) + tuple(x.shape[1:]), dtype=x.dtype, device=x.device)
    out[pd['dst']] = x
    return out


def build_work_list(pads, span_points, tile_points):
    chunk_max = max(GRANULE, tile_points // GRANULE * GRANULE)
    chunks, spans, seg_rec_offs, c_off, spans_per_pair = [], [], [], [0], []
    for m, pd in enumerate(pads):
        first = len(chunks)
        sto = [0]
        for n, (pc, off) in enumerate(zip(pd['pc'], pd['pseg_off'][:-1])):
            k = int(-(-pc // chunk_max))
            if k:
                per = int(-(-(pc // GRANULE) // k)) * GRANULE
                done = 0
                while done < pc:
                    cnt = int(min(per, pc - done))
                    chunks.append((m, n, int(off + done), cnt))
                    done += cnt
            sto.append(4 * (len(chunks) - first))
        seg_rec_offs.append(np.asarray(sto, dtype=np.int32))
        c_off.append(len(chunks))
        ns, q = 0, first
        while q < len(chunks):
            q1, pts = q, 0
            while q1 < len(chunks) and (q1 == q or pts + chunks[q1][3] <= span_points):
                pts += chunks[q1][3]
                q1 += 1
            spans.append((q, q1 - q, pts, m))
            ns += 1
            q = q1
        spans_per_pair.append(ns)
    return dict(chunks=np.asarray(chunks, dtype=np.int32).reshape(-1, 4), spans=np.asarray(spans, dtype=np.int32).reshape(-1, 4),
                seg_rec_offs=seg_rec_offs, c_off=c_off, s_off=np.concatenate(([0], np.cumsum(spans_per_pair))))


_SIDE_STREAMS = {}


class _Layout:
    """A point set with its work list: pix / src4 tables, chunks / spans, per-level descriptors and partial buffers."""


class _Lazy(dict):

    def __init__(self, make, *a, **kw):
        super().__init__(*a, **kw)
        self._make = make

    def __missing__(self, key):
        self[key] = v = self._make(key)
        return v


class PairBatch:
    def __init__(self, src_frames, trg_images, trg_Ks, poses, klds, levels=(0, 3), use_affine=False,
                 tile_points=DEFAULT_BATCH_TILE_POINTS, zmin=1e-7, replicate=1, span_points=None, point_stride=None,
                 extra_tables=(), lazy_levels=True, timer=None, granule=GRANULE, depth_table=True, run_desc=True):
        assert granule in (GRANULE, 64)
        self.granule = int(granule)
        self.rec_per_chunk = 4 if granule == GRANULE else 1
        self.wave_flag = 0 if granule == GRANULE else _lib.SP_COST_WAVE_SPANS
        self.depth_table = bool(depth_table)
        self.table_flag = _lib.SP_COST_DEPTH_TABLE if self.depth_table else 0
        lib = _lib.load()
        self.lib = lib
        M0 = len(src_frames)
        R = int(replicate)
        M = M0 * R
        assert M0 == len(trg_images) == len(trg_Ks) and len(klds) in (M0, M) and poses.shape[0] in (M0, M)
        if poses.shape[0] == M0 and R > 1:
            poses = poses.repeat(R, 1, 1)
        dev = src_frames[0].image.device
        _lib.require_device(src_frames[0].image)
        self.M, self.device = M, dev
        self.level_ids = list(range(levels[0], levels[1]))
        self.tile_points = tile_points
        self.point_stride = {l: 1 for l in self.level_ids}
        if point_stride is not None:
            assert len(point_stride) == len(self.level_ids), "one stride per pyramid level, finest first"
            self.point_stride = {l: int(s) for l, s in zip(self.level_ids, point_stride)}
        coarse_keys = sorted({(l, s) for l, s in self.point_stride.items() if s > 1} | {(int(l), int(s)) for l, s in extra_tables if int(s) > 1})

        klds_all = klds if len(klds) == M and R > 1 else None
        klds = klds[:M0]
        decimated = {l for l, s in coarse_keys if l in self.point_stride and self.point_stride[l] == s}
        full_levels = [l for l in self.level_ids if not (lazy_levels and l in decimated)] or [min(self.level_ids)]
        prep = batch_prepare.prepare_pairs(src_frames, trg_images, trg_Ks, klds, self.level_ids, coarse_keys, dev, full_levels=full_levels,
                                           timer=timer, granule=self.granule, depth_table=self.depth_table)
        self._setup_bytes = prep['bytes']
        self.setup_host_wait_s = prep['host_wait_s']
        mark = timer.mark if timer is not None else (lambda name: None)
        tabs, kp_L, trg, n_off0 = prep['tabs'], prep['kp_L'], prep['trg'], prep['n_off']
        rep = (lambda x: x) if R == 1 else (lambda x: x.repeat(*([R] + [1] * (x.dim() - 1))))
        tile = (lambda a: a) if R == 1 else (lambda a: np.tile(a, R))
        Ns0 = np.diff(n_off0)
        Ns = tile(Ns0)
        n_off = np.concatenate(([0], np.cumsum(Ns)))
        full = tabs[1]
        counts, pc, seg_pos = tile(full.counts), tile(full.pc), tile(full.seg_pos)
        Ppad = tile(np.diff(full.p_off))
        p_off = np.concatenate(([0], np.cumsum(Ppad)))
        self.Ns = Ns.tolist()
        self.Ps = tile(full.points).tolist()
        self.Ppads = Ppad.tolist()
        self.max_N = int(Ns.max())
        self.n_off, self.p_off = n_off, p_off

        self.kp_L = rep(kp_L)
        if klds_all is None:
            self.kld = rep(prep['kld']) if R > 1 else prep['kld']
        else:
            self.kld = torch.cat([batch_prepare._dev(k, dev).reshape(-1) for k in klds_all]).contiguous()
            assert self.kld.numel() == int(n_off[-1]), "one (N_m,) log-depth vector per replicated pair"
        self.pose = poses.detach().to(device=dev, dtype=torch.float32).reshape(M, 16).clone()
        self.aff = torch.zeros(M, 4, dtype=torch.float32, device=dev) if use_affine else None
        self.pix = rep(full.pix)
        sample_full = prep['sample_full']
        self.src4 = _Lazy(lambda l: rep(sample_full([l])[l]).reshape(-1), {l: rep(full.src4[l]).reshape(-1) for l in full_levels})
        self.trg4 = {l: rep(trg[l][0]) for l in self.level_ids}
        trg_off = {l: np.concatenate(([0], np.cumsum(tile(np.diff(trg[l][1]))))) for l in self.level_ids}
        hl_of = {l: np.tile(trg[l][2].astype(np.int32), (R, 1)) for l in self.level_ids}
        self.level_hw = _Lazy(lambda l: list(map(tuple, hl_of[l].tolist())))

        span_div = 1 if self.granule == GRANULE else 4
        if span_points is None:
            span_points = min(DEFAULT_SPAN_POINTS, int(p_off[-1]) // MIN_SPANS) // span_div
        self.span_points = max(int(span_points), self.granule)
        same = lambda a: len(set(self.Ns)) == 1 and bool((np.asarray(a).reshape(M, -1) == np.asarray(a).reshape(M, -1)[0]).all())
        self._uniform_layout = same(pc)
        self.coarse = {}
        specs, spec_of, c_host = [(pc, seg_pos, n_off, self.span_points)], {}, {}
        for l, stride in coarse_keys:
            if stride not in spec_of:
                t = tabs[stride]
                c_pc, c_seg_pos = tile(t.pc), tile(t.seg_pos)
                c_p_off = np.concatenate(([0], np.cumsum(tile(np.diff(t.p_off)))))
                c_span = max(self.granule, min(DEFAULT_SPAN_POINTS, int(c_p_off[-1]) // MIN_SPANS) // span_div)
                spec_of[stride] = len(specs)
                specs.append((c_pc, c_seg_pos, n_off, c_span))
                c_host[stride] = (c_p_off, tile(t.points))
                self._uniform_layout = self._uniform_layout and same(c_pc)
        mark('device arrays')
        lists = batch_prepare.work_lists_staged(specs, tile_points, self.granule, dev)
        mark('work lists')
        wl = lists[0]
        self.chunks, self.spans, self.seg_tile_off = wl['chunks'], wl['spans'], wl['seg_tile_off']
        self.n_chunks, self.n_spans = wl['n_chunks'], wl['n_spans']
        self._s_off = wl['s_off']
        self.span_pair = self.spans[:, 3].long()
        self.n_seg_records = self.rec_per_chunk * self.n_chunks
        coarse_host = {}
        for l, stride in coarse_keys:
            t = tabs[stride]
            lay = _Layout()
            lay.stride = stride
            c_wl = lists[spec_of[stride]]
            c_p_off, c_points = c_host[stride]
            lay.points = c_points.tolist()
            shared = next((o for (l2, s2), o in self.coarse.items() if s2 == stride), None)
            lay.pix = shared.pix if shared is not None else rep(t.pix)
            lay.src4 = rep(t.src4[l]).reshape(-1)
            lay.n_chunks, lay.n_spans = c_wl['n_chunks'], c_wl['n_spans']
            lay.s_off = c_wl['s_off']
            lay.chunks, lay.spans, lay.seg_tile_off = c_wl['chunks'], c_wl['spans'], c_wl['seg_tile_off']
            coarse_host[(l, stride)] = (c_wl, c_p_off)
            self.coarse[(l, stride)] = lay

        Ks = prep['Ks']
        Ks_src, Ks_trg = Ks[:M0], Ks[M0:]
        k4 = lambda K: np.tile(np.stack((K[:, 0, 0], K[:, 1, 1], K[:, 0, 2], K[:, 1, 2]), axis=1).astype(np.float32), (R, 1))
        K4_src, K4_trg = k4(Ks_src), k4(Ks_trg)
        HW = np.tile(prep['shapes'][:, 1:].astype(np.int32), (R, 1))
        pair_idx = np.arange(M, dtype=np.int64)

        kp_L_t, trg4_t, kld_t, pose_t, aff_t = self.kp_L, self.trg4, self.kld, self.pose, self.aff
        pix_t, seg_tile_off_t, Ps_a, rec_per_chunk = self.pix, None, np.asarray(self.Ps), self.rec_per_chunk

        def descriptors(level, pix, src4, seg_tile_off, lay_p_off, lay_wl, real_points):
            d = np.zeros(M, dtype=_SP_PAIR_DTYPE)
            d['pix'] = pix.data_ptr() + 4 * lay_p_off[:-1]
            d['src4'] = src4.data_ptr() + 16 * lay_p_off[:-1]
            d['kp_L'] = kp_L_t.data_ptr() + 4 * n_off[:-1]
            d['trg3'] = trg4_t[level].data_ptr() + 4 * trg_off[level][:-1]
            d['kld'] = kld_t.data_ptr() + 4 * n_off[:-1]
            d['pose'] = pose_t.data_ptr() + 64 * pair_idx
            d['aff'] = (aff_t.data_ptr() + 16 * pair_idx) if use_affine else 0
            d['seg_tile_off'] = seg_tile_off.data_ptr() + 4 * lay_wl['sto_off'][:-1]
            d['K_src'], d['K_trg'] = K4_src, K4_trg
            d['N'], d['P'] = Ns, real_points
            d['H'], d['W'] = HW[:, 0], HW[:, 1]
            d['Hl'], d['Wl'] = hl_of[level][:, 0], hl_of[level][:, 1]
            d['tile0'], d['n_tiles'] = lay_wl['s_off'][:-1], np.diff(lay_wl['s_off'])
            d['zmin'] = zmin
            d['rec0'] = rec_per_chunk * lay_wl['c_off'][:-1]
            return d

        mark('work lists staged')
        self._fine_src = dict(host={s_: (specs[i][0], specs[i][1], c_host[s_][0]) for s_, i in spec_of.items()}, n_off=n_off, descriptors=descriptors,
                              tile_points=tile_points)
        self._fine = {}
        host = [descriptors(l, self.pix, self.src4[l], self.seg_tile_off, p_off, wl, np.asarray(self.Ps)) for l in full_levels]
        for (l, stride), lay in self.coarse.items():
            c_wl, c_p_off = coarse_host[(l, stride)]
            host.append(descriptors(l, lay.pix, lay.src4, lay.seg_tile_off, c_p_off, c_wl, np.maximum(np.asarray(lay.points), 1)))
        mark('descriptors')
        staged = batch_prepare.stage(host, dev)
        src4_d, seg_tile_off_t = self.src4, self.seg_tile_off
        self.desc = _Lazy(lambda l: batch_prepare.stage([descriptors(l, pix_t, src4_d[l], seg_tile_off_t, p_off, wl, Ps_a)], dev)[0],
                          dict(zip(full_levels, staged)))
        by_stride = {}
        for i, lay in enumerate(self.coarse.values()):
            lay.desc = staged[len(full_levels) + i]
            first = by_stride.setdefault(lay.stride, lay)
            if first is lay:
                lay.partials = torch.empty(max(lay.n_spans, 1) * _lib.SP_GN_PARTIAL_FLOATS, dtype=torch.float32, device=dev)
                lay.seg_partials = torch.empty(max(self.rec_per_chunk * lay.n_chunks, 1) * _lib.SP_GN_SEG_FLOATS, dtype=torch.float32, device=dev)
            else:
                lay.partials, lay.seg_partials = first.partials, first.seg_partials

        self.partials = torch.empty(self.n_spans * _lib.SP_GN_PARTIAL_FLOATS, dtype=torch.float32, device=dev)
        self.seg_partials = torch.empty(self.n_seg_records * _lib.SP_GN_SEG_FLOATS, dtype=torch.float32, device=dev)
        widths = (1, 2 + 2 * (self.max_N + 8), _lib.SP_LM_STATE_FLOATS, 16 + self.max_N)
        sizes = [(M * w + 3) // 4 * 4 for w in widths]
        cuts = np.concatenate(([0], np.cumsum(sizes)))
        state_f = torch.zeros(int(cuts[-1]), dtype=torch.float32, device=dev)
        self._costs = state_f[cuts[0]: cuts[0] + M]
        self.adam_state = state_f[cuts[1]: cuts[1] + M * widths[1]].view(M, widths[1])
        self.lm_state = state_f[cuts[2]: cuts[2] + M * widths[2]].view(M, widths[2])
        self.backup = state_f[cuts[3]: cuts[3] + M * widths[3]].view(M, widths[3])
        state_i = torch.zeros(4, M, dtype=torch.int32, device=dev)
        self.arrivals = state_i[0]
        self.done = state_i[1]
        self.phase = state_i[2]
        self.phase_iters = state_i[3]
        mark('workspaces')
        self.reset_lm()
        self._graphs = {}
        self._flags_more = []
        self._flag = None
        self._verdict_arrays = None
        self.status = None
        self.run_desc = None
        if run_desc and self.granule == 64 and self.depth_table:
            n_groups = self.pix.numel() // 64
            rd = torch.empty((n_groups + 1) * 8, dtype=torch.int32, device=dev)
            n_general = torch.zeros(1, dtype=torch.int32, device=dev)
            _lib.check(lib.sp_run_desc_build(_lib.ptr(self.pix), n_groups, _lib.ptr(rd), _lib.ptr(n_general), _lib.stream_ptr()), "sp_run_desc_build")
            if int(n_general.item()) == 0:
                self.run_desc = rd
            mark('run descriptors')
        self._initial = (self.pose.clone(), self.kld.clone())
        mark('constructor returns')

    @property
    def setup_bytes(self):
        if callable(self._setup_bytes):
            self._setup_bytes = self._setup_bytes()
        return self._setup_bytes

    @property
    def seg_records(self):
        return torch.repeat_interleave(self.chunks[:, :2], self.rec_per_chunk, dim=0)

    def restore_initial(self):
        self.pose.copy_(self._initial[0])
        self.kld.copy_(self._initial[1])
        if self.aff is not None:
            self.aff.zero_()
        self.adam_state.zero_()
        self.done.zero_()
        self.phase.zero_()
        self.phase_iters.zero_()
        self.reset_lm()

    @classmethod
    def from_synth(cls, pairs, levels=(0, 3), device="cuda:0", **kw):
        from ..image.keyframe import KeyFrame
        dev = torch.device(device)
        t = lambda a: torch.from_numpy(np.ascontiguousarray(a)).to(dev)
        src = [KeyFrame(t(p.src_image), t(p.K), t(p.logdepth_perseg), t(p.keypoints), t(p.keypoint_regions)) for p in pairs]
        return cls(src, [t(p.trg_image) for p in pairs], [t(p.K) for p in pairs],
                   torch.stack([t(p.pose_init) for p in pairs]), [t(p.kld_init) for p in pairs], levels=levels, **kw)

    def reset_lm(self, lam=1e-4):
        self._lam0 = float(lam)
        self.lm_state.zero_()
        self.lm_state[:, 0] = lam
        self.lm_state[:, 1] = -1.0

    def cost_pass(self, level, mode, irls_eps=1e-3, done=None):
        if mode not in (0, 1) and self.table_flag:
            raise ValueError("cost mode 2 reads log-depth tables: build the batch with depth_table=False")
        rd = self.run_desc is not None and mode in (0, 1)
        _lib.check(self.lib.sp_pairs_cost_opt(_lib.ptr(self.desc[level]), _lib.ptr(self.chunks), _lib.ptr(self.spans), self.n_spans,
                                              mode | self.wave_flag | (self.table_flag if mode in (0, 1) else 0), float(irls_eps), _lib.ptr(self.partials),
                                              _lib.ptr(self.seg_partials), _lib.ptr(done), _lib.ptr(self.pix if rd else None),
                                              _lib.ptr(self.run_desc if rd else None), _lib.stream_ptr()), "sp_pairs_cost_opt")

    def gn_step(self, level=0, irls_eps=1e-3, lm_up=8.0, lm_down=0.5, lm_min=1e-7, fused=False, conv_tol=0.0):
        if fused:
            assert not self.wave_flag and not self.table_flag, "the single-launch form has no wave-span / depth-table variant (PairBatch(depth_table=False))"
            _lib.check(self.lib.sp_pairs_gn_iterate(_lib.ptr(self.desc[level]), _lib.ptr(self.chunks), _lib.ptr(self.spans), self.n_spans, self.M,
                                                    self.max_N, float(irls_eps), _lib.ptr(self.partials), _lib.ptr(self.seg_partials), _lib.ptr(self.arrivals),
                                                    float(lm_up), float(lm_down), float(lm_min), _lib.ptr(self.lm_state),
                                                    _lib.ptr(self.backup), _lib.ptr(self._costs), _lib.stream_ptr()),
                       "sp_pairs_gn_iterate")
            return self._costs
        if conv_tol > 0.0:
            self.cost_pass(level, 1, irls_eps, done=self.done)
            _lib.check(self.lib.sp_pairs_gn_step_conv(_lib.ptr(self.desc[level]), self.M, self.max_N, _lib.ptr(self.partials),
                                                      _lib.ptr(self.seg_partials), float(lm_up), float(lm_down), float(lm_min),
                                                      _lib.ptr(self.lm_state), _lib.ptr(self.backup), _lib.ptr(self._costs),
                                                      float(conv_tol), _lib.ptr(self.done), _lib.stream_ptr()), "sp_pairs_gn_step_conv")
            return self._costs
        self.cost_pass(level, 1, irls_eps)
        return self.solve_gn(level, lm_up, lm_down, lm_min)

    def solve_gn(self, level=0, lm_up=8.0, lm_down=0.5, lm_min=1e-7):
        _lib.check(self.lib.sp_pairs_gn_step(_lib.ptr(self.desc[level]), self.M, self.max_N, _lib.ptr(self.partials), _lib.ptr(self.seg_partials),
                                             float(lm_up), float(lm_down), float(lm_min), _lib.ptr(self.lm_state),
                                             _lib.ptr(self.backup), _lib.ptr(self._costs), _lib.stream_ptr()),
                   "sp_pairs_gn_step")
        return self._costs

    def adam_step(self, level=0, lr_kld=1e-3, lr_pose=1e-2, lr_aff=5e-3, fused=False):
        if fused:
            assert not self.wave_flag and not self.table_flag, "the single-launch form has no wave-span / depth-table variant (PairBatch(depth_table=False))"
            _lib.check(self.lib.sp_pairs_adam_iterate(_lib.ptr(self.desc[level]), _lib.ptr(self.chunks), _lib.ptr(self.spans), self.n_spans, self.M,
                                                      self.max_N, _lib.ptr(self.partials), _lib.ptr(self.seg_partials), _lib.ptr(self.arrivals),
                                                      float(lr_kld), float(lr_pose), float(lr_aff), _lib.ptr(self.adam_state),
                                                      _lib.ptr(self._costs), _lib.stream_ptr()), "sp_pairs_adam_iterate")
            return self._costs
        self.cost_pass(level, 0)
        return self.solve_adam(level, lr_kld, lr_pose, lr_aff)

    def solve_adam(self, level=0, lr_kld=1e-3, lr_pose=1e-2, lr_aff=5e-3):
        _lib.check(self.lib.sp_pairs_adam_step(_lib.ptr(self.desc[level]), self.M, self.max_N, _lib.ptr(self.partials), _lib.ptr(self.seg_partials),
                                               float(lr_kld), float(lr_pose), float(lr_aff), _lib.ptr(self.adam_state),
                                               _lib.ptr(self._costs), _lib.stream_ptr()), "sp_pairs_adam_step")
        return self._costs

    def evaluate(self, level=0):
        self.cost_pass(level, 0)
        p = self.partials[: self.n_spans * _lib.SP_GRAD_PARTIAL_FLOATS].reshape(self.n_spans, _lib.SP_GRAD_PARTIAL_FLOATS)
        sums = torch.zeros(self.M, dtype=torch.float64, device=self.device).index_add_(0, self.span_pair, p[:, 0].double())
        P = torch.tensor(self.Ps, dtype=torch.float64, device=self.device)
        return (sums / (3.0 * P)).float()

    def graph(self, level, mode="gn", iters=1, **kw):
        step = self.gn_step if mode == "gn" else self.adam_step
        step(level, **kw)
        torch.cuda.synchronize()
        g = torch.cuda.CUDAGraph()
        with torch.cuda.graph(g):
            for _ in range(iters):
                step(level, **kw)
        return g

    def run_converging(self, max_iters_per_level=25, conv_tol=1e-3, polish_max=15, polish_eps=1e-5, polish_tol=1e-5, check_every=3, predicted_exit=False, **kw):
        launched = []
        phases = [(level, max_iters_per_level, kw.get("irls_eps", 1e-3), conv_tol) for level in reversed(self.level_ids)]
        if polish_max > 0:
            phases.append((min(self.level_ids), polish_max, polish_eps, polish_tol))
        for level, n_max, eps, tol in phases:
            self.lm_state[:, 1] = -1.0
            self.lm_state[:, 4] = 0.0
            self.done.zero_()
            it = 0
            while it < n_max:
                for _ in range(min(check_every, n_max - it)):
                    self.gn_step(level, **{**kw, "irls_eps": eps, "conv_tol": tol})
                    it += 1
                if bool(self.done.all()):
                    break
            launched.append(it)
        self.done.zero_()
        return launched

    def schedule(self, max_iters_per_level=25, conv_tol=1e-3, polish_max=15, polish_eps=1e-5, polish_tol=1e-5, irls_eps=1e-3, phases=None,
                 use_coarse=True, pose_first_iters=0, pose_first_eps=None, joint_levels=None, use_levels=None, retry_pose_first=None,
                 retry_phases=None, retry_join=None, depth_damp=None, coarse_damped=None, retry2_phases=None, retry2_join=None,
                 adam_lr_pose=ADAM_LR_POSE, adam_lr_kld=ADAM_LR_KLD, predicted_exit=False):
        if phases is None:
            phases = []
            caps = tuple(pose_first_iters) if isinstance(pose_first_iters, (tuple, list)) else ((int(pose_first_iters),) if pose_first_iters > 0 else ())
            coarse_first = sorted(self.level_ids, reverse=True)
            if use_levels is not None:
                coarse_first = coarse_first[len(coarse_first) - int(use_levels):]
            assert len(caps) <= len(coarse_first)
            for level, cap in zip(coarse_first, caps):
                phases.append(dict(level=level, stride=self.point_stride[level] if use_coarse else 1, max_iters=int(cap),
                                   irls_eps=irls_eps if pose_first_eps is None else pose_first_eps, conv_tol=conv_tol, pose_only=True))
            joint = coarse_first if joint_levels is None else coarse_first[len(coarse_first) - int(joint_levels):]
            damps = dict(zip(joint, depth_damp)) if depth_damp else {}
            if coarse_damped == "auto":
                coarse_damped = self.auto_coarse_damping(joint[0], self.point_stride[joint[0]] if use_coarse else 1)
            if coarse_damped:
                phases.append(dict(level=joint[0], stride=self.point_stride[joint[0]] if use_coarse else 1, max_iters=int(coarse_damped[1]), irls_eps=irls_eps,
                                   conv_tol=conv_tol, depth_damp=float(coarse_damped[0])))
            phases += [dict(level=level, stride=self.point_stride[level] if use_coarse else 1, max_iters=max_iters_per_level, irls_eps=irls_eps,
                           conv_tol=conv_tol, depth_damp=damps.get(level, 0.0)) for level in joint]
            finest = min(self.level_ids)
            if polish_max > 0:
                phases.append(dict(level=finest, stride=1, max_iters=polish_max, irls_eps=polish_eps, conv_tol=polish_tol))
            elif use_coarse and self.point_stride[finest] > 1:
                raise ValueError("the finest level iterates on a decimated lattice (point_stride > 1): the schedule needs its all-points polish "
                                 "(polish_max > 0), or use_coarse=False")
        if retry_phases is None and retry_pose_first:
            retry_phases = [dict(level=int(l), stride=self.point_stride[int(l)] if use_coarse else 1, max_iters=int(cap),
                                 irls_eps=irls_eps if pose_first_eps is None else pose_first_eps, conv_tol=conv_tol, pose_only=True)
                            for l, cap in retry_pose_first]
        retry_phases = list(retry_phases or [])
        if retry_phases:
            if retry_join is None:
                retry_join = next((i for i, ph in enumerate(phases) if not ph.get("pose_only", False)), 0)
            assert 0 <= int(retry_join) < len(phases)
        retry2_phases = list(retry2_phases or [])
        if retry2_phases:
            if retry2_join is None:
                retry2_join = max(0, len(phases) - 2)
            assert 0 <= int(retry2_join) < len(phases)
        all_phases = retry2_phases + retry_phases + list(phases)
        if len(all_phases) > _lib.SP_MAX_PHASES:
            raise ValueError(f"{len(all_phases)} phases exceed SP_MAX_PHASES = {_lib.SP_MAX_PHASES}")
        sched = _lib.SpSchedule()
        for p, spec in enumerate(all_phases):
            level, stride = int(spec["level"]), int(spec.get("stride", 1))
            ph = sched.phase[p]
            if stride == 1:
                ph.pairs, ph.chunks, ph.spans, ph.n_spans = _lib.ptr(self.desc[level]), _lib.ptr(self.chunks), _lib.ptr(self.spans), self.n_spans
                ph.span_partials, ph.seg_partials = _lib.ptr(self.partials), _lib.ptr(self.seg_partials)
            else:
                lay = self.fine_layout(level, stride) if spec.get("adam", False) and spec.get("fine_spans", True) and hasattr(self, "_fine_src") else self.coarse[(level, stride)]
                ph.pairs, ph.chunks, ph.spans, ph.n_spans = _lib.ptr(lay.desc), _lib.ptr(lay.chunks), _lib.ptr(lay.spans), lay.n_spans
                ph.span_partials, ph.seg_partials = _lib.ptr(lay.partials), _lib.ptr(lay.seg_partials)
            ph.irls_eps, ph.conv_tol, ph.max_iters = float(spec.get("irls_eps", irls_eps)), float(spec["conv_tol"]), int(spec["max_iters"])
            damp = int(round(8.0 * float(spec.get("depth_damp", 0.0))))
            if not 0 <= damp <= 255:
                raise ValueError("depth_damp: 0 .. 31.875 in steps of 1/8")
            ph.flags = ((_lib.SP_PHASE_POSE_ONLY if spec.get("pose_only", False) else 0) | (_lib.SP_PHASE_WAVE_SPANS if self.wave_flag else 0)
                        | (_lib.SP_PHASE_DEPTH_TABLE if self.table_flag else 0) | (damp << _lib.SP_PHASE_DEPTH_DAMP_SHIFT)
                        | (_lib.SP_PHASE_ADAM if spec.get("adam", False) else 0)
                        | (_lib.SP_PHASE_PREDICTED_EXIT if spec.get("predicted_exit", predicted_exit) else 0))
            ph.next = 0
        n2, n1 = len(retry2_phases), len(retry_phases)
        sched.n_phases = len(all_phases)
        sched.entry = n2 + n1
        sched.retry_entry = -1
        sched.retry2_entry = -1
        if retry_phases:
            sched.retry_entry = n2
            join = n2 + n1 + int(retry_join)
            sched.phase[n2 + n1 - 1].next = join if join != n2 + n1 else 0
        if retry2_phases:
            sched.retry2_entry = 0
            sched.phase[n2 - 1].next = n2 + n1 + int(retry2_join)
            if sched.phase[n2 - 1].next == n2:
                sched.phase[n2 - 1].next = 0
        sched.adam_lr_pose, sched.adam_lr_kld = float(adam_lr_pose), float(adam_lr_kld)
        sched.adam_state = self.adam_state.data_ptr() if any(spec.get("adam", False) for spec in all_phases) else None
        return sched

    FINE_SPAN_POINTS = 512

    def fine_layout(self, level, stride):
        key = (int(level), int(stride))
        if key in self._fine:
            return self._fine[key]
        lay = self.coarse[key]
        first = next((f for (l2, s2), f in self._fine.items() if s2 == key[1]), None)
        src = self._fine_src
        if first is None:
            pc, seg_pos, c_p_off = src['host'][key[1]]
            fine = max(self.granule, self.FINE_SPAN_POINTS)
            wl = batch_prepare.work_lists_staged([(pc, seg_pos, src['n_off'], fine)], fine, self.granule, self.device)[0]
        else:
            wl, c_p_off = first.wl, first.c_p_off
        f = _Layout()
        f.stride, f.wl, f.c_p_off = key[1], wl, c_p_off
        f.chunks, f.spans, f.seg_tile_off, f.n_chunks, f.n_spans, f.s_off = wl['chunks'], wl['spans'], wl['seg_tile_off'], wl['n_chunks'], wl['n_spans'], wl['s_off']
        f.desc = batch_prepare.stage([src['descriptors'](key[0], lay.pix, lay.src4, f.seg_tile_off, c_p_off, wl, np.maximum(np.asarray(lay.points), 1))], self.device)[0]
        if first is None:
            f.partials = torch.empty(max(f.n_spans, 1) * _lib.SP_GN_PARTIAL_FLOATS, dtype=torch.float32, device=self.device)
            f.seg_partials = torch.empty(max(self.rec_per_chunk * f.n_chunks, 1) * _lib.SP_GN_SEG_FLOATS, dtype=torch.float32, device=self.device)
        else:
            f.partials, f.seg_partials = first.partials, first.seg_partials
        self._fine[key] = f
        return f

    def auto_coarse_damping(self, level, stride):
        pts = np.asarray(self.Ps if stride == 1 else self.coarse[(level, stride)].points, dtype=np.float64)
        per_seg = float(np.median(pts / np.maximum(np.asarray(self.Ns, dtype=np.float64), 1.0)))
        return (16.0, 12) if per_seg >= 48.0 else (12.0, 12)

    def _verdict(self, sched, verdict):
        if verdict is False:
            self.status = None
            return None
        opt = dict(VERDICT_DEFAULTS, **(verdict if isinstance(verdict, dict) else {}))
        if getattr(self, "_verdict_arrays", None) is None:
            ints = torch.zeros(2, self.M, dtype=torch.int32, device=self.device)
            self._verdict_arrays = (ints[0], ints[1], torch.zeros(self.M, _lib.SP_DIAG_FLOATS, dtype=torch.float32, device=self.device),
                                    torch.empty_like(self.pose), torch.empty_like(self.kld))
        status, attempts, diag, pose0, kld0 = self._verdict_arrays
        status.zero_(); attempts.zero_(); diag.zero_()
        pose0.copy_(self.pose); kld0.copy_(self.kld)
        v = _lib.SpVerdict()
        v.status, v.diag, v.attempts = status.data_ptr(), diag.data_ptr(), attempts.data_ptr()
        v.pose0, v.kld0, v.pose_base, v.kld_base = pose0.data_ptr(), kld0.data_ptr(), self.pose.data_ptr(), self.kld.data_ptr()
        v.kld_bound, v.cost_bound, v.cost_ratio, v.valid_min = float(opt["kld_bound"]), float(opt["cost_bound"]), float(opt["cost_ratio"]), float(opt["valid_min"])
        v.retry_mask = int(opt["retry_on"]) if (sched.retry_entry >= 0 or sched.retry2_entry >= 0) else 0
        v.lam0 = float(getattr(self, "_lam0", 1e-4))
        v.seg_max_ratio, v.seg_mean_ratio, v.seg_product = float(opt["seg_max_ratio"]), float(opt["seg_mean_ratio"]), float(opt["seg_product"])
        self.evals = None
        if opt.get("count_evaluations", False):
            self.evals = torch.zeros(self.M, _lib.SP_MAX_PHASES, dtype=torch.int32, device=self.device)
            v.evals = self.evals.data_ptr()
        self.status, self.attempts, self.diag = status, attempts, diag
        return v

    def failed(self):
        if getattr(self, "status", None) is None:
            raise RuntimeError("no verdict: run_scheduled(verdict=False), or no scheduled run yet")
        return (self.status & _lib.SP_STATUS_FAILED) != 0

    def run_scheduled(self, check_every=4, lm_up=8.0, lm_down=0.5, lm_min=1e-7, slots=None, verdict=None, return_status=False, streams=1, **schedule_kw):
        sched = self.schedule(**schedule_kw)
        tail = sum(sched.phase[p].max_iters for p in range(sched.entry, sched.n_phases))
        bound = sum(sched.phase[p].max_iters for p in range(sched.n_phases)) + tail * ((sched.retry_entry >= 0) + (sched.retry2_entry >= 0))
        if self._flag is None:
            self._flag = (torch.zeros(8, dtype=torch.int32, device=self.device), torch.zeros(8, dtype=torch.int32).pin_memory())
        v = self._verdict(sched, verdict)
        v_addr = ctypes.addressof(v) if v is not None else None
        outlier = float(dict(VERDICT_DEFAULTS, **(verdict if isinstance(verdict, dict) else {}))["cost_outlier"]) if v is not None else 0.0
        if sched.adam_state:
            self.adam_state.zero_()
        if slots is not None and int(slots) < self.M:
            it = self._run_queue(sched, int(slots), bound, check_every, lm_up, lm_down, lm_min, v, v_addr, streams=streams, schedule_kw=schedule_kw)
            if outlier > 0.0 and self.M >= COST_OUTLIER_MIN_PAIRS:
                it += self._cost_outlier_pass(outlier, v, bound, check_every, lm_up, lm_down, lm_min, schedule_kw)
            return (it, self.status) if return_status else it
        self.phase.fill_(sched.entry)
        self.phase_iters.zero_()
        self.lm_state[:, 1] = -1.0
        self.lm_state[:, 4:] = 0.0
        it = self.lib.sp_pairs_schedule_run(ctypes.addressof(sched), self.M, self.max_N, float(lm_up), float(lm_down), float(lm_min),
                                            _lib.ptr(self.lm_state), _lib.ptr(self.backup), _lib.ptr(self._costs), _lib.ptr(self.phase),
                                            _lib.ptr(self.phase_iters), int(check_every), int(bound), _lib.ptr(self._flag[0]),
                                            self._flag[1].data_ptr(), v_addr, _lib.stream_ptr())
        if it < 0:
            _lib.check(it if it > -1000 else -(it + 1000), "sp_pairs_schedule_run")
        if outlier > 0.0 and self.M >= COST_OUTLIER_MIN_PAIRS:
            it += self._cost_outlier_pass(outlier, v, bound, check_every, lm_up, lm_down, lm_min, schedule_kw)
        return (it, self.status) if return_status else it

    def _cost_outlier_pass(self, factor, v, bound, check_every, lm_up, lm_down, lm_min, schedule_kw):
        F, M = _lib.SP_STATUS_FAILED, self.M
        cost = self.diag[:, 0]
        clean = ((self.status & F) == 0) & torch.isfinite(cost) & (cost > 0)
        n_clean = int(clean.sum())
        if n_clean < COST_OUTLIER_MIN_PAIRS:
            return 0
        bound_c = factor * cost[clean].median()
        it = 0
        sched = self.schedule(**schedule_kw)
        entries = [e for e in (sched.retry_entry, sched.retry2_entry) if e >= 0]
        for _ in range(len(entries)):
            out = (self.diag[:, 0] > bound_c) & ((self.status & F) == 0)
            nxt = torch.full_like(self.attempts, -1)
            if sched.retry_entry >= 0:
                nxt = torch.where(self.attempts == 0, 1, nxt)
            if sched.retry2_entry >= 0:
                nxt = torch.where((self.attempts == 1) | ((self.attempts == 0) & (nxt < 0)), 2, nxt)
            again = out & (nxt > 0)
            if not bool(again.any()):
                break
            if getattr(self, "_seg_pair", None) is None:
                self._seg_pair = torch.repeat_interleave(torch.arange(M, device=self.device), torch.as_tensor(self.Ns, device=self.device))
            pose0, kld0 = self._verdict_arrays[3], self._verdict_arrays[4]
            self.pose.copy_(torch.where(again[:, None], pose0, self.pose))
            self.kld.copy_(torch.where(again[self._seg_pair], kld0, self.kld))
            self.attempts.copy_(torch.where(again, nxt, self.attempts))
            entry = torch.where(nxt == 1, sched.retry_entry, sched.retry2_entry)
            self.phase.copy_(torch.where(again, entry, sched.n_phases).to(torch.int32))
            self.phase_iters.zero_()
            ls = self.lm_state
            ls[:, 0] = torch.where(again, float(getattr(self, "_lam0", 1e-4)), ls[:, 0])
            ls[:, 1] = torch.where(again, -1.0, ls[:, 1])
            ls[:, 4:] = torch.where(again[:, None], 0.0, ls[:, 4:])
            self.diag[:, 5] = torch.where(again, 0.0, self.diag[:, 5])
            if sched.adam_state:
                self.adam_state.zero_()
            n = self.lib.sp_pairs_schedule_run(ctypes.addressof(sched), M, self.max_N, float(lm_up), float(lm_down), float(lm_min),
                                               _lib.ptr(self.lm_state), _lib.ptr(self.backup), _lib.ptr(self._costs), _lib.ptr(self.phase),
                                               _lib.ptr(self.phase_iters), int(check_every), int(bound), _lib.ptr(self._flag[0]),
                                               self._flag[1].data_ptr(), ctypes.addressof(v), _lib.stream_ptr())
            if n < 0:
                _lib.check(n if n > -1000 else -(n + 1000), "sp_pairs_schedule_run")
            it += n
        out = (self.diag[:, 0] > bound_c) & ((self.status & F) == 0)
        self.status.bitwise_or_(out.to(torch.int32) * _lib.SP_STATUS_COST)
        return it

    def _run_queue(self, sched, slots, bound, check_every, lm_up, lm_down, lm_min, v, v_addr, streams=1, schedule_kw=None):
        assert slots >= 1
        M, dev = self.M, self.device
        rec = ctypes.sizeof(_lib.SpPair)
        lam0 = float(getattr(self, "_lam0", 1e-4))
        wave = bool(self.wave_flag)
        most = lambda s_off: int(np.diff(np.asarray(s_off)).max())
        spans_of = {_lib.ptr(self.spans).value: most(self._s_off)}
        for lay in list(self.coarse.values()) + list(getattr(self, "_fine", {}).values()):
            spans_of[_lib.ptr(lay.spans).value] = most(lay.s_off)
        n_groups = max(1, min(int(streams), slots))
        cuts = [slots * g // n_groups for g in range(n_groups + 1)]
        head = torch.tensor([slots], dtype=torch.int32, device=dev)
        slot_pair = torch.arange(slots, dtype=torch.int32, device=dev)
        active = torch.zeros(slots, dtype=torch.int32, device=dev)
        q_costs = torch.zeros(M, dtype=torch.float32, device=dev)
        q_lm = torch.zeros(M, _lib.SP_LM_STATE_FLOATS, dtype=torch.float32, device=dev)
        self.phase.fill_(sched.n_phases)
        self.phase[:slots] = sched.entry
        self.phase_iters.zero_()
        self.lm_state.zero_()
        self.lm_state[:, 0] = lam0
        self.lm_state[:, 1] = -1.0
        rounds = bound * (-(-M // slots) + 1)
        while len(self._flags_more) < n_groups - 1:
            self._flags_more.append((torch.zeros(8, dtype=torch.int32, device=dev), torch.zeros(8, dtype=torch.int32).pin_memory()))
        flags = [self._flag] + self._flags_more[: n_groups - 1]
        keep, groups = [], []
        for g in range(n_groups):
            lo, n_g = cuts[g], cuts[g + 1] - cuts[g]
            sg = sched if g == 0 else self.schedule(**(schedule_kw or {}))
            q = _lib.SpQueue()
            slot_desc = {}
            for p in range(sg.n_phases):
                ph = sg.phase[p]
                full_ptr = ph.pairs
                if full_ptr not in slot_desc:
                    full = next(t for t in list(self.desc.values()) + [lay.desc for lay in list(self.coarse.values()) + list(getattr(self, "_fine", {}).values())]
                                if t.data_ptr() == full_ptr)
                    slot_desc[full_ptr] = full[lo * rec: (lo + n_g) * rec].clone()
                    keep.append(full)
                q.qpairs[p] = full_ptr
                q.slot_pairs[p] = slot_desc[full_ptr].data_ptr()
                ph.pairs = slot_desc[full_ptr].data_ptr()
                ms = spans_of[ph.spans] if ph.n_spans > 0 else 0
                q.max_spans[p] = (ms + 3) // 4 * 4 if wave else ms
            q.n_queue, q.head, q.slot_pair, q.q_costs, q.q_lm, q.lam0 = M, head.data_ptr(), slot_pair[lo:].data_ptr(), q_costs.data_ptr(), q_lm.data_ptr(), lam0
            q.active = active[lo:].data_ptr()
            if sg.adam_state:
                sg.adam_state = self.adam_state[lo:].data_ptr()
            keep.append(slot_desc)
            keep.append(active)
            groups.append((sg, q, lo, n_g))

        def drive(g, stream):
            sg, q, lo, n_g = groups[g]
            return self.lib.sp_pairs_schedule_run_queue(ctypes.addressof(sg), ctypes.addressof(q), n_g, self.max_N, float(lm_up), float(lm_down),
                                                        float(lm_min), _lib.ptr(self.lm_state[lo:]), _lib.ptr(self.backup[lo:]), _lib.ptr(self._costs[lo:]),
                                                        _lib.ptr(self.phase[lo:]), _lib.ptr(self.phase_iters[lo:]), int(check_every), int(rounds),
                                                        _lib.ptr(flags[g][0]), flags[g][1].data_ptr(), v_addr, stream)

        if n_groups == 1:
            its = [drive(0, _lib.stream_ptr())]
        else:
            import threading
            main = torch.cuda.current_stream()
            pool = _SIDE_STREAMS.setdefault(dev, [])
            while len(pool) < n_groups - 1:
                pool.append(torch.cuda.Stream(device=dev))
            side = pool[: n_groups - 1]
            its = [0] * n_groups
            for st in side:
                st.wait_stream(main)

            def work(g):
                torch.cuda.set_device(dev)
                its[g] = drive(g, ctypes.c_void_p(side[g - 1].cuda_stream))

            threads = [threading.Thread(target=work, args=(g,)) for g in range(1, n_groups)]
            for t in threads:
                t.start()
            its[0] = drive(0, _lib.stream_ptr())
            for t in threads:
                t.join()
            for st in side:
                main.wait_stream(st)
        for it in its:
            if it < 0:
                _lib.check(it if it > -1000 else -(it + 1000), "sp_pairs_schedule_run_queue")
        it = max(its)
        min_phase = min(int(f[1][0]) for f in flags)
        taken = min(max(int(f[1][1]) for f in flags), M)
        self._costs.copy_(q_costs)
        self.lm_state.copy_(q_lm)
        self._queue_stats = dict(slots=slots, head=taken, slot_pair=slot_pair, finished=min_phase >= sched.n_phases, rounds_by_stream=list(its))
        if min_phase < sched.n_phases:
            if v is None:
                raise RuntimeError(f"run_scheduled(slots={slots}) ended on its round limit ({rounds}) with pairs unfinished")
            self.status[taken:] = _lib.SP_STATUS_UNFINISHED
        self.phase.fill_(sched.n_phases)
        return it

    def run(self, iters_per_level, mode="gn", use_graph=False, polish_iters=0, polish_eps=1e-5, **kw):
        self._run_levels(iters_per_level, mode, use_graph, **kw)
        if mode == "gn" and polish_iters > 0:
            finest = min(self.level_ids)
            for _ in range(polish_iters):
                self.gn_step(finest, **{**kw, "irls_eps": polish_eps})

    def _run_levels(self, iters_per_level, mode, use_graph, **kw):
        per_level = isinstance(iters_per_level, (tuple, list))
        if per_level:
            assert len(iters_per_level) == len(self.level_ids)
        for li, level in enumerate(reversed(self.level_ids)):
            n_iters = iters_per_level[li] if per_level else iters_per_level
            if mode == "gn":
                self.lm_state[:, 1] = -1.0
                self.lm_state[:, 4] = 0.0
            if use_graph:
                key = (level, mode, tuple(sorted(kw.items())))
                g = self._graphs.get(key)
                done = 0
                if g is None:
                    g = self._graphs[key] = self.graph(level, mode, 1, **kw)
                    done = 1
                for _ in range(n_iters - done):
                    g.replay()
            else:
                for _ in range(n_iters):
                    (self.gn_step if mode == "gn" else self.adam_step)(level, **kw)

    def costs(self):
        return self._costs

    def poses(self):
        return self.pose.reshape(self.M, 4, 4)

    def klds(self):
        return [self.kld[self.n_off[m]: self.n_off[m + 1]] for m in range(self.M)]

    def schedule_traffic(self, **schedule_kw):
        assert getattr(self, "evals", None) is not None, "run_scheduled(verdict=dict(count_evaluations=True)) first"
        sched = self.schedule(**schedule_kw)
        ev = self.evals.cpu().numpy().astype(np.float64)
        where = {self.desc[l].data_ptr(): (l, 1) for l in list(self.desc.keys())}
        where.update({lay.desc.data_ptr(): key for key, lay in self.coarse.items()})
        where.update({lay.desc.data_ptr(): key for key, lay in getattr(self, "_fine", {}).items()})
        phases, total = [], 0.0
        for p in range(sched.n_phases):
            level, stride = where[sched.phase[p].pairs]
            pts = np.asarray(self.Ps if stride == 1 else self.coarse[(level, stride)].points, dtype=np.float64)
            hw = np.asarray(self.level_hw[level], dtype=np.float64)
            per_pair = 20.0 * pts + 12.0 * hw[:, 0] * hw[:, 1]
            fl = sched.phase[p].flags
            kind = ("adam" if fl & _lib.SP_PHASE_ADAM else "pose-only" if fl & _lib.SP_PHASE_POSE_ONLY else
                    "damped" if (fl >> _lib.SP_PHASE_DEPTH_DAMP_SHIFT) & 0xff else "joint")
            if p == sched.n_phases - 1 and stride == 1:
                kind = "polish"
            nbytes = float((ev[:, p] * per_pair).sum())
            total += nbytes
            phases.append(dict(phase=p, level=int(level), stride=int(stride), kind=kind, attempt=("third" if p < max(sched.retry_entry, 0) and sched.retry2_entry >= 0 else
                                                                                                   "second" if p < sched.entry else "first"),
                               evaluations=int(ev[:, p].sum()), bytes=nbytes, bytes_per_evaluation=float(per_pair.mean())))
        return dict(total_bytes=total, evaluations=int(ev.sum()), phases=phases)

    def algorithmic_bytes(self, level):
        return sum(20 * P + 12 * h * w for P, (h, w) in zip(self.Ps, self.level_hw[level]))
```

Measured before the change: 453,000 iters/s.

## Keep the accepted GN system so rejected LM steps re-solve without re-reducing partials

When a Levenberg-Marquardt step is accepted, the per-pair normal-equation column sums and per-segment sums are now stored in a double-precision side buffer. When the next step is rejected, the same launch restores the backup and immediately re-solves with the larger damping from that buffer. Previously it returned and spent an extra iteration re-evaluating the cost. This removes a full cost/grad pass per rejection and also skips the per-tile segment re-reductions. In exchange every accepted step writes the kept system to global memory, adding extra stores and per-pair storage.

```diff
diff --git a/include/sp_hip.h b/include/sp_hip.h
--- a/include/sp_hip.h
+++ b/include/sp_hip.h
@@ -175,6 +175,8 @@
 #define SP_PHASE_DEPTH_DAMP(k) (((k) & 0xff) << SP_PHASE_DEPTH_DAMP_SHIFT)
 #define SP_PHASE_ADAM 8
 #define SP_PHASE_PREDICTED_EXIT 16
+#define SP_PHASE_KEEP_SYSTEM 32
+#define SP_KEPT_SYSTEM_DOUBLES(max_N) (32 + 10 * (max_N))
 typedef struct SpPhase {
     const SpPair* pairs;
     const int32_t* chunks;
@@ -236,9 +238,17 @@
                               float* lm_state, float* backup, float* costs, int32_t* phase, int32_t* iters, const SpVerdict* verdict ,
                               void* stream);
 
+int sp_pairs_schedule_gn_step_keep(const SpSchedule* sched, int n_pairs, int max_N, float lm_up, float lm_down, float lm_min,
+                                   float* lm_state, float* backup, float* costs, int32_t* phase, int32_t* iters, const SpVerdict* verdict ,
+                                   double* kept, void* stream);
+
 int sp_pairs_schedule_run(const SpSchedule* sched, int n_pairs, int max_N, float lm_up, float lm_down, float lm_min,
                           float* lm_state, float* backup, float* costs, int32_t* phase, int32_t* iters, int check_every,
                           int max_rounds, int32_t* flag_dev, int32_t* flag_host, const SpVerdict* verdict , void* stream);
+
+int sp_pairs_schedule_run_keep(const SpSchedule* sched, int n_pairs, int max_N, float lm_up, float lm_down, float lm_min,
+                               float* lm_state, float* backup, float* costs, int32_t* phase, int32_t* iters, int check_every,
+                               int max_rounds, int32_t* flag_dev, int32_t* flag_host, const SpVerdict* verdict , double* kept, void* stream);
 
 typedef struct SpQueue {
     const SpPair* qpairs[SP_MAX_PHASES];
@@ -258,6 +268,11 @@
                                 float lm_min, float* lm_state, float* backup, float* costs, int32_t* phase, int32_t* iters,
                                 int check_every, int max_rounds, int32_t* flag_dev, int32_t* flag_host, const SpVerdict* verdict ,
                                 void* stream);
+
+int sp_pairs_schedule_run_queue_keep(const SpSchedule* sched, const SpQueue* queue, int n_slots, int max_N, float lm_up, float lm_down,
+                                     float lm_min, float* lm_state, float* backup, float* costs, int32_t* phase, int32_t* iters,
+                                     int check_every, int max_rounds, int32_t* flag_dev, int32_t* flag_host, const SpVerdict* verdict ,
+                                     double* kept, void* stream);
 
 int sp_pairs_adam_iterate(const SpPair* pairs, const int32_t* chunks, const int32_t* spans, int n_spans, int n_pairs, int max_N,
                           float* span_partials, float* seg_partials, int32_t* arrivals, float lr_kld, float lr_pose, float lr_aff, float* state,
diff --git a/super_primitive_amd/_lib.py b/super_primitive_amd/_lib.py
--- a/super_primitive_amd/_lib.py
+++ b/super_primitive_amd/_lib.py
@@ -44,6 +44,9 @@
     "sp_pairs_schedule_gn_step": [P, I, I, F, F, F, P, P, P, P, P, P, P],
     "sp_pairs_schedule_run": [P, I, I, F, F, F, P, P, P, P, P, I, I, P, P, P, P],
     "sp_pairs_schedule_run_queue": [P, P, I, I, F, F, F, P, P, P, P, P, I, I, P, P, P, P],
+    "sp_pairs_schedule_gn_step_keep": [P, I, I, F, F, F, P, P, P, P, P, P, P, P],
+    "sp_pairs_schedule_run_keep": [P, I, I, F, F, F, P, P, P, P, P, I, I, P, P, P, P, P],
+    "sp_pairs_schedule_run_queue_keep": [P, P, I, I, F, F, F, P, P, P, P, P, I, I, P, P, P, P, P],
     "sp_pairs_adam_iterate": [P, P, P, I, I, I, P, P, P, F, F, F, P, P, P],
     "sp_pairs_gn_iterate": [P, P, P, I, I, I, F, P, P, P, F, F, F, P, P, P, P],
     "sp_window_scratch_doubles": [I, I],
@@ -112,6 +115,11 @@
 SP_PHASE_DEPTH_TABLE = 4
 SP_PHASE_ADAM = 8
 SP_PHASE_PREDICTED_EXIT = 16
+SP_PHASE_KEEP_SYSTEM = 32
+
+
+def kept_system_doubles(max_N):
+    return 32 + 10 * int(max_N)
 SP_PHASE_DEPTH_DAMP_SHIFT = 8
 SP_PREP_DEPTH_TABLE = 0x10000
 SP_PREP_DENSE_L = 0x20000
diff --git a/super_primitive_amd/csrc/sp_solve_device.h b/super_primitive_amd/csrc/sp_solve_device.h
--- a/super_primitive_amd/csrc/sp_solve_device.h
+++ b/super_primitive_amd/csrc/sp_solve_device.h
@@ -182,41 +182,57 @@
 
 #define SP_SEG_CACHE 256
 
-__device__ __forceinline__ void segment_system(const float* __restrict__ p, const int32_t* __restrict__ seg_tile_off, int n,
-                                               double lam, double (&o)[8], bool pose_only = false) {
+template <int NC>
+__device__ __forceinline__ void segment_sums(const float* __restrict__ p, const int32_t* __restrict__ seg_tile_off, int n, double (&o)[NC]) {
+    static_assert(NC == 8 || NC == 10, "8: the normal equations' columns; 10: with the cost columns");
     constexpr int NV = SP_GN_SEG_FLOATS;
-    if (pose_only) {
-#pragma unroll
-        for (int i = 0; i < 8; ++i) o[i] = 0.0;
-        return;
-    }
-    double h[6] = {0, 0, 0, 0, 0, 0}, D = 0.0, bd = 0.0;
+    double s[NC];
+#pragma unroll
+    for (int i = 0; i < NC; ++i) s[i] = 0.0;
     const int t0 = seg_tile_off[n], t1 = seg_tile_off[n + 1];
     for (int t = t0; t < t1; t += 8) {
-        float v[8][8];
+        float v[8][NC];
 #pragma unroll
         for (int u = 0; u < 8; ++u) {
             const float4* q = reinterpret_cast<const float4*>(p + (size_t)min(t + u, t1 - 1) * NV);
             const float4 a = q[0], b = q[1];
             v[u][0] = a.x; v[u][1] = a.y; v[u][2] = a.z; v[u][3] = a.w;
             v[u][4] = b.x; v[u][5] = b.y; v[u][6] = b.z; v[u][7] = b.w;
+            if constexpr (NC == 10) {
+                const float2 c = *reinterpret_cast<const float2*>(q + 2);
+                v[u][8] = c.x; v[u][9] = c.y;
+            }
         }
 #pragma unroll
         for (int u = 0; u < 8; ++u) {
             if (t + u < t1) {
 #pragma unroll
-                for (int i = 0; i < 6; ++i) h[i] += (double)v[u][i];
-                D += (double)v[u][6];
-                bd += (double)v[u][7];
-            }
-        }
-    }
-    const double Dd = D * (1.0 + lam);
-#pragma unroll
-    for (int i = 0; i < 6; ++i) o[i] = h[i];
+                for (int i = 0; i < NC; ++i) s[i] += (double)v[u][i];
+            }
+        }
+    }
+#pragma unroll
+    for (int i = 0; i < NC; ++i) o[i] = s[i];
+}
+
+__device__ __forceinline__ void segment_damp(double (&o)[8], double lam) {
+    const double Dd = o[6] * (1.0 + lam);
     o[6] = Dd > 1e-12 ? 1.0 / Dd : 0.0;
-    o[7] = bd;
-}
+}
+
+__device__ __forceinline__ void segment_system(const float* __restrict__ p, const int32_t* __restrict__ seg_tile_off, int n,
+                                               double lam, double (&o)[8], bool pose_only = false) {
+    if (pose_only) {
+#pragma unroll
+        for (int i = 0; i < 8; ++i) o[i] = 0.0;
+        return;
+    }
+    segment_sums<8>(p, seg_tile_off, n, o);
+    segment_damp(o, lam);
+}
+
+#define SP_KEPT_HEAD 32
+#define SP_KEPT_SEG 10
 
 struct GnArgs {
     int max_N;
@@ -236,6 +252,8 @@
     float* adam_state;
     int predicted_exit;
     uint32_t idle_mask;
+    double* kept;
+    int keep;
 };
 
 __device__ __forceinline__ void leave_phase(const GnArgs& h, int pi, float* __restrict__ ls, int spent, bool on_cap) {
@@ -245,7 +263,8 @@
     ls[7] = on_cap ? (float)spent : -(float)spent;
 }
 
-__device__ __forceinline__ void solve_gn(const SpPair* __restrict__ pairs, int pi, const float* __restrict__ partials,
+template <bool KEEP = false>
+__device__ __forceinline__ bool solve_gn(const SpPair* __restrict__ pairs, int pi, const float* __restrict__ partials,
                                          const float* __restrict__ seg_partials, const GnArgs& h) {
     const int max_N = h.max_N;
     const float lm_up = h.lm_up, lm_down = h.lm_down, lm_min = h.lm_min;
@@ -261,14 +280,17 @@
     __shared__ double dxi[6];
     __shared__ double gain_part[SP_WAVES];
     __shared__ int decision;
+    __shared__ int resolve;
     const SpPair& pr = pairs[pi];
-    if (h.done && h.done[pi]) return;
+    if (h.done && h.done[pi]) return false;
     const float* p = partials + (size_t)pr.tile0 * NV;
     const float* sp = seg_partials + (size_t)pr.rec0 * SP_GN_SEG_FLOATS;
     float* ls = lm_state + (size_t)pi * SP_LM_STRIDE;
     float* bk = backup + (size_t)pi * (16 + max_N);
+    double* kp = nullptr;
+    if constexpr (KEEP) { if (h.keep && h.kept) kp = h.kept + (size_t)pi * (SP_KEPT_HEAD + SP_KEPT_SEG * (size_t)max_N); }
     reduce_columns<NV>(p, pr.n_tiles, sums, scratch);
-    const double cost = sums[0] / (3.0 * (double)pr.P);
+    double cost = sums[0] / (3.0 * (double)pr.P);
     if (threadIdx.x == 0) {
         const float last = ls[1];
         int rej = 0;
@@ -279,34 +301,80 @@
             if (h.phase) { leave_phase(h, pi, ls, h.iters[pi], false); ls[4] = 0.f; }
         }
         decision = rej;
+        if constexpr (KEEP) resolve = 0;
         ls[5] = (float)cost;
         ls[6] = (float)(sums[28] / (double)pr.P);
         costs[pi] = (float)cost;
     }
     __syncthreads();
-    if (decision == 2) return;
+    if (decision == 2) return false;
+    bool from_kept = false;
     if (decision == 1) {
         for (int i = threadIdx.x; i < 16; i += SP_BLOCK) pr.pose[i] = bk[i];
         for (int n = threadIdx.x; n < pr.N; n += SP_BLOCK) pr.kld[n] = bk[16 + n];
         if (threadIdx.x == 0) {
+            bool ended = false;
             ls[0] *= lm_up; ls[3] += 1.f; ls[4] = 1.f;
             if (h.phase) {
                 const int n = h.iters[pi] + 1;
-                if (n >= h.max_iters) { leave_phase(h, pi, ls, n, true); ls[4] = 0.f; }
+                if (n >= h.max_iters) { leave_phase(h, pi, ls, n, true); ls[4] = 0.f; ended = true; }
                 else h.iters[pi] = n;
             }
-        }
-        return;
+            if constexpr (KEEP) resolve = (kp && !ended) ? 1 : 0;
+        }
+        if constexpr (!KEEP) return false;
+        else {
+            if (!kp) return false;
+            __syncthreads();
+            if (!resolve) return false;
+            from_kept = true;
+            if (threadIdx.x < 29) sums[threadIdx.x] = kp[threadIdx.x];
+            __syncthreads();
+            cost = sums[0] / (3.0 * (double)pr.P);
+            if (threadIdx.x == 0) {
+                ls[5] = (float)cost;
+                ls[6] = (float)(sums[28] / (double)pr.P);
+                costs[pi] = (float)cost;
+            }
+        }
     }
     float lambda = ls[0];
     if (ls[4] == 0.f) lambda = fmaxf(lambda * lm_down, lm_min);
     const double lam = (double)lambda;
-    for (int i = threadIdx.x; i < 16; i += SP_BLOCK) bk[i] = pr.pose[i];
-    for (int n = threadIdx.x; n < pr.N; n += SP_BLOCK) bk[16 + n] = pr.kld[n];
+    const double lam_d = lam + (double)h.depth_damp;
+    const bool pose_only = h.pose_only != 0;
+    if (!from_kept) {
+        for (int i = threadIdx.x; i < 16; i += SP_BLOCK) bk[i] = pr.pose[i];
+        for (int n = threadIdx.x; n < pr.N; n += SP_BLOCK) bk[16 + n] = pr.kld[n];
+        if constexpr (KEEP) {
+            if (kp) {
+                if (threadIdx.x < 29) kp[threadIdx.x] = sums[threadIdx.x];
+                for (int n = threadIdx.x; n < pr.N; n += SP_BLOCK) {
+                    double r[SP_KEPT_SEG];
+                    segment_sums<SP_KEPT_SEG>(sp, pr.seg_tile_off, n, r);
+                    double* k = kp + SP_KEPT_HEAD + (size_t)SP_KEPT_SEG * n;
+#pragma unroll
+                    for (int i = 0; i < SP_KEPT_SEG; ++i) k[i] = r[i];
+                }
+            }
+        }
+    }
+    auto system_of = [&](int n, double (&o)[8]) {
+        if constexpr (KEEP) {
+            if (kp) {
+                const double* k = kp + SP_KEPT_HEAD + (size_t)SP_KEPT_SEG * n;
+#pragma unroll
+                for (int i = 0; i < 8; ++i) o[i] = pose_only ? 0.0 : k[i];
+                if (!pose_only) segment_damp(o, lam_d);
+                return;
+            }
+        }
+        segment_system(sp, pr.seg_tile_off, n, lam_d, o, pose_only);
+    };
     const int n_cached = min(pr.N, SP_SEG_CACHE);
     for (int n = threadIdx.x; n < n_cached; n += SP_BLOCK) {
         double o[8];
-        segment_system(sp, pr.seg_tile_off, n, lam + (double)h.depth_damp, o, h.pose_only != 0);
+        system_of(n, o);
 #pragma unroll
         for (int i = 0; i < 8; ++i) seg[n][i] = o[i];
     }
@@ -323,7 +391,7 @@
                 if (n < SP_SEG_CACHE) {
 #pragma unroll
                     for (int i = 0; i < 8; ++i) o[i] = seg[n][i];
-                } else segment_system(sp, pr.seg_tile_off, n, lam + (double)h.depth_damp, o, h.pose_only != 0);
+                } else system_of(n, o);
                 acc += o[a] * (k < 21 ? o[b] : o[7]) * o[6];
             }
             schur_part[j][k] = acc;
@@ -359,7 +427,7 @@
         if (n < SP_SEG_CACHE) {
 #pragma unroll
             for (int i = 0; i < 8; ++i) o[i] = seg[n][i];
-        } else segment_system(sp, pr.seg_tile_off, n, lam + (double)h.depth_damp, o, h.pose_only != 0);
+        } else system_of(n, o);
         if (o[6] > 0.0) {
             double r = -o[7];
 #pragma unroll
@@ -393,6 +461,7 @@
             else h.iters[pi] = n;
         }
     }
+    return from_kept;
 }
 
 __device__ __forceinline__ void solve_adam_sched(const SpPair* __restrict__ pairs, int pi, const float* __restrict__ partials,
diff --git a/super_primitive_amd/csrc/sp_solver.hip b/super_primitive_amd/csrc/sp_solver.hip
--- a/super_primitive_amd/csrc/sp_solver.hip
+++ b/super_primitive_amd/csrc/sp_solver.hip
@@ -14,6 +14,7 @@
 
 static_assert(sizeof(SpPhase) == 64 && sizeof(SpSchedule) == 800 && sizeof(SpVerdict) == 104 && sizeof(SpQueue) == 296 && sizeof(SpPair) == 136,
               "SpSchedule / SpVerdict / SpQueue / SpPair are part of the ABI");
+static_assert(SP_KEPT_SYSTEM_DOUBLES(3) == SP_KEPT_HEAD + SP_KEPT_SEG * 3, "the kept system's layout (sp_solve_device.h) is the header's size");
 
 __global__ __launch_bounds__(SP_BLOCK) void k_pairs_gn_sched(SpSchedule sched, GnArgs h, SpQueue q, SpVerdict v, const int32_t* __restrict__ active) {
     const int slot = active ? active[blockIdx.x] : blockIdx.x;
@@ -21,6 +22,7 @@
     if (ph >= sched.n_phases || ph < 0) return;
     if ((h.idle_mask >> ph) & 1u) return;
     if (v.evals && threadIdx.x == 0) v.evals[(size_t)(q.n_queue > 0 ? q.slot_pair[slot] : slot) * SP_MAX_PHASES + ph] += 1;
+    bool resolved = false;
     {
         const SpPhase& s = sched.phase[ph];
         h.conv_tol = s.conv_tol;
@@ -30,8 +32,9 @@
         h.depth_damp = 0.125f * (float)((s.flags >> SP_PHASE_DEPTH_DAMP_SHIFT) & 0xff);
         h.adam_lr_pose = sched.adam_lr_pose; h.adam_lr_kld = sched.adam_lr_kld; h.adam_state = sched.adam_state;
         h.predicted_exit = s.flags & SP_PHASE_PREDICTED_EXIT;
+        h.keep = s.flags & SP_PHASE_KEEP_SYSTEM;
         if ((s.flags & SP_PHASE_ADAM) && sched.adam_state) solve_adam_sched(s.pairs, slot, s.span_partials, s.seg_partials, h);
-        else solve_gn(s.pairs, slot, s.span_partials, s.seg_partials, h);
+        else resolved = solve_gn<true>(s.pairs, slot, s.span_partials, s.seg_partials, h);
     }
     if (q.n_queue <= 0 && !v.status) return;
     __shared__ int next_s, retry_s;
@@ -65,9 +68,11 @@
         int sn = 0;
         {
             const float* sp = sched.phase[ph].seg_partials + (size_t)pr.rec0 * SP_GN_SEG_FLOATS;
+            const double* kseg = resolved ? h.kept + (size_t)slot * (SP_KEPT_HEAD + SP_KEPT_SEG * (size_t)h.max_N) + SP_KEPT_HEAD : nullptr;
             for (int n = threadIdx.x; n < n_seg; n += SP_BLOCK) {
                 double a = 0.0, c = 0.0;
-                for (int t = pr.seg_tile_off[n]; t < pr.seg_tile_off[n + 1]; ++t) {
+                if (kseg) { a = kseg[(size_t)SP_KEPT_SEG * n + 8]; c = kseg[(size_t)SP_KEPT_SEG * n + 9]; }
+                else for (int t = pr.seg_tile_off[n]; t < pr.seg_tile_off[n + 1]; ++t) {
                     a += (double)sp[(size_t)t * SP_GN_SEG_FLOATS + 8];
                     c += (double)sp[(size_t)t * SP_GN_SEG_FLOATS + 9];
                 }
@@ -270,7 +275,7 @@
     return m;
 }
 
-static int check_schedule(const SpSchedule* sched, const SpVerdict* v) {
+static int check_schedule(const SpSchedule* sched, const SpVerdict* v, const double* kept = nullptr) {
     if (!sched || sched->n_phases <= 0 || sched->n_phases > SP_MAX_PHASES) return SP_EINVAL;
     if (sched->entry < 0 || sched->entry >= sched->n_phases || sched->retry_entry < -1 || sched->retry_entry >= sched->n_phases) return SP_EINVAL;
     if (sched->retry2_entry < -1 || sched->retry2_entry >= sched->n_phases) return SP_EINVAL;
@@ -279,6 +284,7 @@
         if (!ph.pairs || !ph.span_partials || !ph.seg_partials || ph.max_iters <= 0) return SP_EINVAL;
         if ((ph.flags & SP_PHASE_ADAM) && (!sched->adam_state || !(sched->adam_lr_pose > 0.f) || !(sched->adam_lr_kld > 0.f))) return SP_EINVAL;
         if (ph.next != 0 && (ph.next <= p || ph.next > sched->n_phases)) return SP_EINVAL;
+        if ((ph.flags & SP_PHASE_KEEP_SYSTEM) && !(ph.flags & SP_PHASE_ADAM) && !kept) return SP_EINVAL;
     }
     if (v && v->status) {
         if (!v->pose0 || !v->kld0 || !v->pose_base || !v->kld_base) return SP_EINVAL;
@@ -287,24 +293,32 @@
     return 0;
 }
 
+int sp_pairs_schedule_gn_step_keep(const SpSchedule* sched, int n_pairs, int max_N, float lm_up, float lm_down, float lm_min,
+                                   float* lm_state, float* backup, float* costs, int32_t* phase, int32_t* iters, const SpVerdict* verdict,
+                                   double* kept, void* stream) {
+    if (!sched || !lm_state || !backup || !costs || !phase || !iters || n_pairs <= 0 || max_N <= 0) return SP_EINVAL;
+    if (int rc = check_schedule(sched, verdict, kept)) return rc;
+    GnArgs ga{max_N, lm_up, lm_down, lm_min, lm_state, backup, costs, 0.f, nullptr, phase, iters, 0, 0, 0};
+    ga.kept = kept;
+    hipLaunchKernelGGL(k_pairs_gn_sched, dim3(n_pairs), dim3(SP_BLOCK), 0, static_cast<hipStream_t>(stream), *sched, ga, SpQueue{},
+                       verdict ? *verdict : SpVerdict{}, (const int32_t*)nullptr);
+    SP_CHECK_LAUNCH();
+    return 0;
+}
+
 int sp_pairs_schedule_gn_step(const SpSchedule* sched, int n_pairs, int max_N, float lm_up, float lm_down, float lm_min,
                               float* lm_state, float* backup, float* costs, int32_t* phase, int32_t* iters, const SpVerdict* verdict,
                               void* stream) {
-    if (!sched || !lm_state || !backup || !costs || !phase || !iters || n_pairs <= 0 || max_N <= 0) return SP_EINVAL;
-    if (int rc = check_schedule(sched, verdict)) return rc;
-    hipLaunchKernelGGL(k_pairs_gn_sched, dim3(n_pairs), dim3(SP_BLOCK), 0, static_cast<hipStream_t>(stream), *sched,
-                       GnArgs{max_N, lm_up, lm_down, lm_min, lm_state, backup, costs, 0.f, nullptr, phase, iters, 0, 0, 0}, SpQueue{},
-                       verdict ? *verdict : SpVerdict{}, (const int32_t*)nullptr);
-    SP_CHECK_LAUNCH();
-    return 0;
-}
-
-int sp_pairs_schedule_run_queue(const SpSchedule* sched, const SpQueue* queue, int n_slots, int max_N, float lm_up, float lm_down,
-                                float lm_min, float* lm_state, float* backup, float* costs, int32_t* phase, int32_t* iters,
-                                int check_every, int max_rounds, int32_t* flag_dev, int32_t* flag_host, const SpVerdict* verdict, void* stream) {
+    return sp_pairs_schedule_gn_step_keep(sched, n_pairs, max_N, lm_up, lm_down, lm_min, lm_state, backup, costs, phase, iters, verdict, nullptr, stream);
+}
+
+int sp_pairs_schedule_run_queue_keep(const SpSchedule* sched, const SpQueue* queue, int n_slots, int max_N, float lm_up, float lm_down,
+                                     float lm_min, float* lm_state, float* backup, float* costs, int32_t* phase, int32_t* iters,
+                                     int check_every, int max_rounds, int32_t* flag_dev, int32_t* flag_host, const SpVerdict* verdict,
+                                     double* kept, void* stream) {
     if (!sched || !queue || !phase || !iters || !flag_dev || !flag_host || !lm_state || !backup || !costs) return SP_EINVAL;
     if (check_every <= 0 || max_rounds < 0 || n_slots <= 0 || max_N <= 0 || queue->n_queue < n_slots) return SP_EINVAL;
-    if (int rc = check_schedule(sched, verdict)) return rc;
+    if (int rc = check_schedule(sched, verdict, kept)) return rc;
     if (!queue->head || !queue->slot_pair || !queue->q_costs || !queue->q_lm) return SP_EINVAL;
     for (int p = 0; p < sched->n_phases; ++p) {
         const SpPhase& ph = sched->phase[p];
@@ -330,6 +344,7 @@
         const uint32_t idle = adam_mask & ~occupied;
         GnArgs ga{max_N, lm_up, lm_down, lm_min, lm_state, backup, costs, 0.f, nullptr, phase, iters, 0, 0, 0};
         ga.idle_mask = idle;
+        ga.kept = kept;
         for (int k = 0; k < n; ++k, ++it) {
             int rc = schedule_cost_from(sched, phase, stream, reached, queue, n_slots, tail ? queue->active : nullptr, tail ? n_active : 0, idle);
             if (rc != 0) return rc < 0 ? rc : -(1000 + rc);
@@ -361,12 +376,19 @@
     return it;
 }
 
-int sp_pairs_schedule_run(const SpSchedule* sched, int n_pairs, int max_N, float lm_up, float lm_down, float lm_min,
-                          float* lm_state, float* backup, float* costs, int32_t* phase, int32_t* iters, int check_every,
-                          int max_rounds, int32_t* flag_dev, int32_t* flag_host, const SpVerdict* verdict, void* stream) {
+int sp_pairs_schedule_run_queue(const SpSchedule* sched, const SpQueue* queue, int n_slots, int max_N, float lm_up, float lm_down,
+                                float lm_min, float* lm_state, float* backup, float* costs, int32_t* phase, int32_t* iters,
+                                int check_every, int max_rounds, int32_t* flag_dev, int32_t* flag_host, const SpVerdict* verdict, void* stream) {
+    return sp_pairs_schedule_run_queue_keep(sched, queue, n_slots, max_N, lm_up, lm_down, lm_min, lm_state, backup, costs, phase, iters, check_every,
+                                            max_rounds, flag_dev, flag_host, verdict, nullptr, stream);
+}
+
+int sp_pairs_schedule_run_keep(const SpSchedule* sched, int n_pairs, int max_N, float lm_up, float lm_down, float lm_min,
+                               float* lm_state, float* backup, float* costs, int32_t* phase, int32_t* iters, int check_every,
+                               int max_rounds, int32_t* flag_dev, int32_t* flag_host, const SpVerdict* verdict, double* kept, void* stream) {
     if (!sched || !phase || !iters || !flag_dev || !flag_host || check_every <= 0 || max_rounds < 0) return SP_EINVAL;
     if (!lm_state || !backup || !costs || n_pairs <= 0 || max_N <= 0) return SP_EINVAL;
-    if (int rc = check_schedule(sched, verdict)) return rc;
+    if (int rc = check_schedule(sched, verdict, kept)) return rc;
     hipStream_t s = static_cast<hipStream_t>(stream);
     const bool may_retry = verdict && verdict->status && verdict->attempts && verdict->retry_mask != 0 && (sched->retry_entry >= 0 || sched->retry2_entry >= 0);
     const int last_attempt = sched->retry2_entry >= 0 ? 2 : 1;
@@ -380,10 +402,11 @@
         const uint32_t idle = adam_mask & ~occupied;
         for (int k = 0; k < n; ++k, ++it) {
             int rc = schedule_cost_from(sched, phase, stream, reached, nullptr, 0, nullptr, 0, idle);
-            if (rc == 0) rc = check_schedule(sched, verdict);
+            if (rc == 0) rc = check_schedule(sched, verdict, kept);
             if (rc != 0) return rc < 0 ? rc : -(1000 + rc);
             GnArgs ga{max_N, lm_up, lm_down, lm_min, lm_state, backup, costs, 0.f, nullptr, phase, iters, 0, 0, 0};
             ga.idle_mask = idle;
+            ga.kept = kept;
             hipLaunchKernelGGL(k_pairs_gn_sched, dim3(n_pairs), dim3(SP_BLOCK), 0, s, *sched, ga, SpQueue{}, verdict ? *verdict : SpVerdict{}, (const int32_t*)nullptr);
             hipError_t el = hipGetLastError();
             if (el != hipSuccess) return -(1000 + (int)el);
@@ -408,6 +431,13 @@
     return it;
 }
 
+int sp_pairs_schedule_run(const SpSchedule* sched, int n_pairs, int max_N, float lm_up, float lm_down, float lm_min,
+                          float* lm_state, float* backup, float* costs, int32_t* phase, int32_t* iters, int check_every,
+                          int max_rounds, int32_t* flag_dev, int32_t* flag_host, const SpVerdict* verdict, void* stream) {
+    return sp_pairs_schedule_run_keep(sched, n_pairs, max_N, lm_up, lm_down, lm_min, lm_state, backup, costs, phase, iters, check_every, max_rounds,
+                                      flag_dev, flag_host, verdict, nullptr, stream);
+}
+
 int sp_pairs_gn_step(const SpPair* pairs, int n_pairs, int max_N, const float* partials, const float* seg_partials,
                      float lm_up, float lm_down, float lm_min, float* lm_state, float* backup, float* costs, void* stream) {
     return sp_pairs_gn_step_conv(pairs, n_pairs, max_N, partials, seg_partials, lm_up, lm_down, lm_min, lm_state, backup, costs, 0.f,
diff --git a/super_primitive_amd/optim/pair_batch.py b/super_primitive_amd/optim/pair_batch.py
--- a/super_primitive_amd/optim/pair_batch.py
+++ b/super_primitive_amd/optim/pair_batch.py
@@ -283,6 +283,7 @@
         self.adam_state = state_f[cuts[1]: cuts[1] + M * widths[1]].view(M, widths[1])
         self.lm_state = state_f[cuts[2]: cuts[2] + M * widths[2]].view(M, widths[2])
         self.backup = state_f[cuts[3]: cuts[3] + M * widths[3]].view(M, widths[3])
+        self.kept_system = torch.empty(M, _lib.kept_system_doubles(self.max_N), dtype=torch.float64, device=dev)
         state_i = torch.zeros(4, M, dtype=torch.int32, device=dev)
         self.arrivals = state_i[0]
         self.done = state_i[1]
@@ -435,7 +436,7 @@
     def schedule(self, max_iters_per_level=25, conv_tol=1e-3, polish_max=15, polish_eps=1e-5, polish_tol=1e-5, irls_eps=1e-3, phases=None,
                  use_coarse=True, pose_first_iters=0, pose_first_eps=None, joint_levels=None, use_levels=None, retry_pose_first=None,
                  retry_phases=None, retry_join=None, depth_damp=None, coarse_damped=None, retry2_phases=None, retry2_join=None,
-                 adam_lr_pose=ADAM_LR_POSE, adam_lr_kld=ADAM_LR_KLD, predicted_exit=False):
+                 adam_lr_pose=ADAM_LR_POSE, adam_lr_kld=ADAM_LR_KLD, predicted_exit=False, keep_rejected_system=False):
         if phases is None:
             phases = []
             caps = tuple(pose_first_iters) if isinstance(pose_first_iters, (tuple, list)) else ((int(pose_first_iters),) if pose_first_iters > 0 else ())
@@ -496,7 +497,8 @@
             ph.flags = ((_lib.SP_PHASE_POSE_ONLY if spec.get("pose_only", False) else 0) | (_lib.SP_PHASE_WAVE_SPANS if self.wave_flag else 0)
                         | (_lib.SP_PHASE_DEPTH_TABLE if self.table_flag else 0) | (damp << _lib.SP_PHASE_DEPTH_DAMP_SHIFT)
                         | (_lib.SP_PHASE_ADAM if spec.get("adam", False) else 0)
-                        | (_lib.SP_PHASE_PREDICTED_EXIT if spec.get("predicted_exit", predicted_exit) else 0))
+                        | (_lib.SP_PHASE_PREDICTED_EXIT if spec.get("predicted_exit", predicted_exit) else 0)
+                        | (_lib.SP_PHASE_KEEP_SYSTEM if keep_rejected_system and not spec.get("adam", False) else 0))
             ph.next = 0
         n2, n1 = len(retry2_phases), len(retry_phases)
         sched.n_phases = len(all_phases)
@@ -579,7 +581,9 @@
             raise RuntimeError("no verdict: run_scheduled(verdict=False), or no scheduled run yet")
         return (self.status & _lib.SP_STATUS_FAILED) != 0
 
-    def run_scheduled(self, check_every=4, lm_up=8.0, lm_down=0.5, lm_min=1e-7, slots=None, verdict=None, return_status=False, streams=1, **schedule_kw):
+    def run_scheduled(self, check_every=4, lm_up=8.0, lm_down=0.5, lm_min=1e-7, slots=None, verdict=None, return_status=False, streams=1,
+                      keep_rejected_system=True, **schedule_kw):
+        schedule_kw = dict(schedule_kw, keep_rejected_system=bool(keep_rejected_system))
         sched = self.schedule(**schedule_kw)
         tail = sum(sched.phase[p].max_iters for p in range(sched.entry, sched.n_phases))
         bound = sum(sched.phase[p].max_iters for p in range(sched.n_phases)) + tail * ((sched.retry_entry >= 0) + (sched.retry2_entry >= 0))
@@ -599,10 +603,10 @@
         self.phase_iters.zero_()
         self.lm_state[:, 1] = -1.0
         self.lm_state[:, 4:] = 0.0
-        it = self.lib.sp_pairs_schedule_run(ctypes.addressof(sched), self.M, self.max_N, float(lm_up), float(lm_down), float(lm_min),
-                                            _lib.ptr(self.lm_state), _lib.ptr(self.backup), _lib.ptr(self._costs), _lib.ptr(self.phase),
-                                            _lib.ptr(self.phase_iters), int(check_every), int(bound), _lib.ptr(self._flag[0]),
-                                            self._flag[1].data_ptr(), v_addr, _lib.stream_ptr())
+        it = self.lib.sp_pairs_schedule_run_keep(ctypes.addressof(sched), self.M, self.max_N, float(lm_up), float(lm_down), float(lm_min),
+                                                 _lib.ptr(self.lm_state), _lib.ptr(self.backup), _lib.ptr(self._costs), _lib.ptr(self.phase),
+                                                 _lib.ptr(self.phase_iters), int(check_every), int(bound), _lib.ptr(self._flag[0]),
+                                                 self._flag[1].data_ptr(), v_addr, _lib.ptr(self.kept_system), _lib.stream_ptr())
         if it < 0:
             _lib.check(it if it > -1000 else -(it + 1000), "sp_pairs_schedule_run")
         if outlier > 0.0 and self.M >= COST_OUTLIER_MIN_PAIRS:
@@ -646,10 +650,10 @@
             self.diag[:, 5] = torch.where(again, 0.0, self.diag[:, 5])
             if sched.adam_state:
                 self.adam_state.zero_()
-            n = self.lib.sp_pairs_schedule_run(ctypes.addressof(sched), M, self.max_N, float(lm_up), float(lm_down), float(lm_min),
-                                               _lib.ptr(self.lm_state), _lib.ptr(self.backup), _lib.ptr(self._costs), _lib.ptr(self.phase),
-                                               _lib.ptr(self.phase_iters), int(check_every), int(bound), _lib.ptr(self._flag[0]),
-                                               self._flag[1].data_ptr(), ctypes.addressof(v), _lib.stream_ptr())
+            n = self.lib.sp_pairs_schedule_run_keep(ctypes.addressof(sched), M, self.max_N, float(lm_up), float(lm_down), float(lm_min),
+                                                    _lib.ptr(self.lm_state), _lib.ptr(self.backup), _lib.ptr(self._costs), _lib.ptr(self.phase),
+                                                    _lib.ptr(self.phase_iters), int(check_every), int(bound), _lib.ptr(self._flag[0]),
+                                                    self._flag[1].data_ptr(), ctypes.addressof(v), _lib.ptr(self.kept_system), _lib.stream_ptr())
             if n < 0:
                 _lib.check(n if n > -1000 else -(n + 1000), "sp_pairs_schedule_run")
             it += n
@@ -713,10 +717,10 @@
 
         def drive(g, stream):
             sg, q, lo, n_g = groups[g]
-            return self.lib.sp_pairs_schedule_run_queue(ctypes.addressof(sg), ctypes.addressof(q), n_g, self.max_N, float(lm_up), float(lm_down),
-                                                        float(lm_min), _lib.ptr(self.lm_state[lo:]), _lib.ptr(self.backup[lo:]), _lib.ptr(self._costs[lo:]),
-                                                        _lib.ptr(self.phase[lo:]), _lib.ptr(self.phase_iters[lo:]), int(check_every), int(rounds),
-                                                        _lib.ptr(flags[g][0]), flags[g][1].data_ptr(), v_addr, stream)
+            return self.lib.sp_pairs_schedule_run_queue_keep(ctypes.addressof(sg), ctypes.addressof(q), n_g, self.max_N, float(lm_up), float(lm_down),
+                                                             float(lm_min), _lib.ptr(self.lm_state[lo:]), _lib.ptr(self.backup[lo:]), _lib.ptr(self._costs[lo:]),
+                                                             _lib.ptr(self.phase[lo:]), _lib.ptr(self.phase_iters[lo:]), int(check_every), int(rounds),
+                                                             _lib.ptr(flags[g][0]), flags[g][1].data_ptr(), v_addr, _lib.ptr(self.kept_system[lo:]), stream)
 
         if n_groups == 1:
             its = [drive(0, _lib.stream_ptr())]
```

Result: no change. 453,000 iters/s (median of 2 runs) (+0.0%).
